# gligen/GLIGEN

Hardware: AMD Instinct MI355X
Metric: 512x512 images/sec @ 50 PLMS steps, box+text (CFG 7.5), UNet step ms (higher is better)
Workload: dtype bf16; 1 GPU; C2: box+text, 8 boxes (30 grounding tokens), 512x512, 50 PLMS steps, CFG 7.5, bf16 storage / fp32 accumulate; plms_steps=50, unet_evals_per_image=102, hipgraph=True, batches_in_flight=3

## Files before the change

gligen_amd/_lib.py:

```python
from __future__ import annotations

import ctypes as C
from pathlib import Path

_HERE = Path(__file__).resolve().parent
LIB_PATH = _HERE / "libgligen_amd.so"


class GligenAmdError(RuntimeError):
    pass


class UNetConfig(C.Structure):
    _fields_ = [
        ("in_channels", C.c_int), ("out_channels", C.c_int), ("model_channels", C.c_int),
        ("num_res_blocks", C.c_int), ("num_heads", C.c_int), ("context_dim", C.c_int),
        ("n_mult", C.c_int), ("channel_mult", C.c_int * 8),
        ("n_attn", C.c_int), ("attention_resolutions", C.c_int * 8),
        ("inpaint_mode", C.c_int), ("grounding_kind", C.c_int),
        ("gr_in_dim", C.c_int), ("gr_out_dim", C.c_int), ("max_persons", C.c_int), ("fuser_kind", C.c_int),
        ("extra_channels", C.c_int), ("tok_resize", C.c_int), ("tok_in_dim", C.c_int),
    ]


# ... 186 lines not shown
TRAIN_PRIM_SYMBOLS = {
    "gl_op_train_attention": (_I, [_P, _I, _I, _I, _I, _I] + [_P] * 9 + [_P]),
    "gl_op_train_linear": (_I, [_P, _I, _I, _I] + [_P] * 8 + [_P]),
    "gl_op_train_layernorm": (_I, [_P, _I, _I, _F, _P, _P, _P, _P, _I] + [_P] * 6 + [_P]),
    "gl_op_train_groupnorm": (_I, [_P, _I, _I, _I, _I, _F, _P, _P, _P, _P, _I] + [_P] * 4 + [_P]),
    "gl_op_train_geglu": (_I, [_P, _I, _I, _P, _P, _P, _P, _P]),
    "gl_op_train_dot": (_I, [_P, C.c_int64, _P, _P, _P, _F, _I, _P, _P]),
    "gl_op_train_conv3": (_I, [_P] + [_I] * 6 + [_P] * 6 + [_P]),
    "gl_op_train_conv_direct": (_I, [_P] + [_I] * 7 + [_P] * 7 + [_P]),
}

class LoraAdapter(C.Structure):
    _fields_ = [("name", C.c_char_p), ("down", C.c_void_p), ("up", C.c_void_p), ("g_down", C.c_void_p), ("g_up", C.c_void_p), ("rank", C.c_int),
                ("scale", C.c_float)]


TRAIN_LORA_SYMBOLS = {
    "gl_unet_train_step_lora": (_I, [_P, C.POINTER(UNetConfig), C.POINTER(TrainUNetIn), _I, C.POINTER(C.c_char_p), C.POINTER(_P), C.POINTER(_P),
                                     C.POINTER(LoraAdapter), _I, _P, _P, _P]),
    "gl_op_lora_linear": (_I, [_P, _I, _I, _I, _I, _F, _I, _I] + [_P] * 10 + [_P]),
    "gl_lora_wgrad_chunk_rows": (_I, [_I]),
}

TRAIN_LORA_CONV_SYMBOLS = {
    "gl_op_lora_conv3": (_I, [_P, _I, _I, _I, _I, _I, _I, _F, _I] + [_P] * 10 + [_P]),
}

TRAINER_SYMBOLS = {
    "gl_op_adamw_ema_step": (_I, [_P, _P, _P, _P, _P, _P, C.c_int64, C.c_double, C.c_double, C.c_double, C.c_double, C.c_double, C.c_double, _I, _P]),
}

_D = C.c_double
TRAIN_RUN_SYMBOLS = {
    "gl_op_grad_accumulate": (_I, [_P, _P, _P, C.c_int64, _I, _I, _P]),
    "gl_grad_sqnorm_partials": (C.c_int64, [C.c_int64]),
    "gl_op_grad_sqnorm": (_I, [_P, _P, C.c_int64, _P, _P]),
    "gl_op_clip_coef": (_I, [_P, _P, C.c_int64, C.c_float, _P, _P]),
    "gl_op_adamw_clip_step": (_I, [_P, _P, _P, _P, _P, C.c_int64, _D, _D, _D, _D, _D, _I, _P, _P]),
    "gl_op_adamw_ema_clip_step": (_I, [_P, _P, _P, _P, _P, _P, C.c_int64, _D, _D, _D, _D, _D, _D, _I, _P, _P]),
    "gl_train_set_loss_weights": (_I, [_P, _P, _I]),
}
GRAD_ACCUM_MODES = {"first": 0, "middle": 1, "last": 2}

SAMPLER_SYMBOLS = {
    "gl_set_cfg_shared_prefix": (_I, [_I]),
}

SOLVER_SYMBOLS = {
    "gl_sample_solver": (_I, [_P, C.POINTER(SolverArgs), _P]),
    "gl_op_solver_update": (_I, [_P, _P, _I, C.c_float, C.c_float, _P, _P, _P, _P, _P, _P] + [C.c_float] * 5 + [C.c_int64, _P]),
}


class GemmPlanRecord(C.Structure):
    _fields_ = [("kernel", C.c_char * 96)] + [(n, C.c_int) for n in ("family", "M", "N", "K", "tm", "tn", "splits", "grid", "n_items", "box", "rm", "rz",
                                                                     "units_per_split", "xcd")]


class AttnProjLayout(C.Structure):
    _fields_ = [(n, C.c_int) for n in ("d", "dp", "dpv", "tq", "tk", "tq_pad", "tk_pad", "vt_perm32")]


class GemmEpilogueArgs(C.Structure):
    _fields_ = [("struct_size", C.c_uint), ("conv", _I), ("M", _I), ("N", _I), ("K", _I), ("x0", _P), ("x1", _P)] + \
               [(n, _I) for n in ("C0", "C1", "B", "H", "W", "stride", "ups", "pad_lo")] + \
               [("w", _P), ("bias", _P), ("bias2", _P), ("bias2_ld", _I), ("rows_per_b", _I), ("res", _P), ("ldres", _I), ("gate", _P)] + \
               [(n, _I) for n in ("act", "out_f32", "mode", "n_real", "remap_in", "remap_out", "remap_off")] + [("out", _P), ("ldo", _I)]


GEMM_PLAN_SYMBOLS = {
    "gl_op_attention_project_range": (_I, [_P, _P, _I, _I, _I, _I, _I, _P, _P, _P, _P, _P, _P, _P, C.POINTER(AttnProjLayout), _P]),
    "gl_op_gemm_epilogue": (_I, [_P, C.POINTER(GemmEpilogueArgs), _P]),
    "gl_gemm_force_plan": (_I, [_I, _I, _I, _I]),
    "gl_gemm_force_knobs": (_I, [_I, _I, _I, _I, _I, _I]),
    "gl_gemm_force_clear": (_I, []),
    "gl_gemm_plan_log_clear": (_I, []),
    "gl_gemm_plan_log": (_I, [C.POINTER(GemmPlanRecord), _I, C.POINTER(_I), C.POINTER(_I)]),
    "gl_op_attention_project": (_I, [_P, _P, _P, _I, _I, _I, _I, _I, _I, _P, _P, _P, _P, _P, _P, C.POINTER(AttnProjLayout), _P]),
}

ATTENTION_CORE_SYMBOLS = {
    "gl_op_attention_core": (_I, [_P, _P, _P, _P, C.POINTER(AttnProjLayout), _I, _I, _I, _I, _P, _I, _I, _I, _P]),
}
ATTN_CORE_KERNELS = {"auto": 0, "attn_kernel": 1, "attn2_kernel_w4": 2, "attn2_kernel_w8": 3, "attn3_kernel": 4}
GL_ERR_UNSUPPORTED = 5


class FFRowsArgs(C.Structure):
    _fields_ = [("struct_size", C.c_uint), ("M", _I), ("C", _I), ("x", _P), ("ldx", _I), ("normalize", _I), ("eps", C.c_float), ("gamma", _P), ("beta", _P),
                ("w1", _P), ("b1", _P), ("w2", _P), ("b2", _P), ("res", _P), ("ldres", _I), ("gate", _P), ("out", _P), ("ldo", _I), ("stats_out", _P),
                ("stats_ld", _I), ("pre", _I), ("post", _I), ("pre_w", _P), ("pre_b", _P), ("pre_res", _P), ("ld_pre_res", _I), ("pre_gate", _P),
                ("mid_out", _P), ("ld_mid", _I), ("post_w", _P), ("post_b", _P), ("post_res", _P), ("ld_post_res", _I), ("gamma_q", _P), ("beta_q", _P),
                ("q", _P), ("qDP", _I), ("qT", _I), ("qTpad", _I)]


class QkvRowsArgs(C.Structure):
    _fields_ = [("struct_size", C.c_uint), ("M", _I), ("C", _I), ("H", _I), ("x", _P), ("ldx", _I), ("normalize", _I), ("eps", C.c_float), ("pre", _I),
                ("pre_w", _P), ("pre_b", _P), ("pre_res", _P), ("ld_pre_res", _I), ("mid_out", _P), ("ld_mid", _I), ("stats_out", _P), ("gamma", _P),
                ("beta", _P), ("np", _I), ("w", _P), ("bias", _P), ("q", _P), ("k", _P), ("vt", _P), ("DP", _I), ("DPV", _I), ("T", _I), ("Tpad_q", _I),
                ("Tpad_k", _I), ("in_period", _I)]


FFN_ROWS_SYMBOLS = {
    "gl_op_ff_rows": (_I, [_P, C.POINTER(FFRowsArgs), _P]),
    "gl_op_qkv_rows": (_I, [_P, C.POINTER(QkvRowsArgs), _P]),
}

class LayerNormRowsArgs(C.Structure):
    _fields_ = [("struct_size", C.c_uint), ("x", _P), ("x2", _P), ("B", _I), ("N1", _I), ("N2", _I), ("Tpad", _I), ("C", _I), ("eps", C.c_float),
                ("gamma", _P), ("beta", _P), ("y", _P), ("ldx", _I), ("ldy", _I)]


NORM_SYMBOLS = {
    "gl_op_groupnorm_coef": (_I, [_P, _P, _I, _P, _I, _I, _I, _P, _P, C.c_float, _P, C.POINTER(_I), _P]),
    "gl_op_layernorm_rows": (_I, [_P, C.POINTER(LayerNormRowsArgs), _P]),
}

VAE_SYMBOLS = {
    "gl_vae_set_attention": (_I, [_P, _I]),
    "gl_op_vae_attention": (_I, [_P, _P, _P, _P, _I, _I, _I, _I, _P, _P]),
}
VAE_ATTN_MODES = {"auto": 0, "matrix": 1, "flash": 2}

LATENT_SYMBOLS = {
    "gl_op_latent_renoise": (_I, [_P, _P, _I, _I, _I, _I, _P, _I, _I, _I, _F, _F, _P, _I, _P]),
    "gl_latent_resize_taps": (_I, [_I, _I, _I, C.POINTER(_I), C.POINTER(_F)]),
}
LATENT_RESIZE_MODES = {"nearest-exact": 0, "bilinear": 1, "bicubic": 2}

LORA_SYMBOLS = {
    "gl_op_lora_merge": (_I, [_P, _P, _P, _P, _I, _I, _I, _F, _P]),
}



class TilePlan(C.Structure):
    _fields_ = [("struct_size", C.c_uint)] + [(n, C.c_int) for n in ("ny", "nx", "th_in", "tw_in", "th_out", "tw_out")] + \
               [(n, C.c_void_p) for n in ("windows", "oy", "ox", "wy", "wx")]


TILING_SYMBOLS = {
    "gl_vae_decode_tiled": (_I, [_P, _I, _I, _I, _P, _P, C.POINTER(TilePlan), _I, _P]),
    "gl_vae_encode_tiled": (_I, [_P, _I, _I, _I, _P, _P, _P, _P, C.POINTER(TilePlan), _I, _P]),
    "gl_op_tile_gather": (_I, [_P, _P, _I, _I, _I, _I, _P, _I, _P, _I, _I, _P]),
    "gl_op_tile_blend": (_I, [_P, _P, _I, _I, C.POINTER(TilePlan), _P, _I, _I, _I, _I, _P]),
}

FUSER_KINDS = {"gatedSA": 0, "gatedSA2": 1, "gatedCA": 2}


def fuser_kind(fuser_type) -> int:
    try:
        return FUSER_KINDS[fuser_type or "gatedSA"]
    except KeyError:
        raise ValueError(f"fuser_type {fuser_type!r}: one of {sorted(FUSER_KINDS)}") from None


_lib = None


def load() -> C.CDLL:
    global _lib
    if _lib is not None:
        return _lib
    if not LIB_PATH.exists():
        raise GligenAmdError(
            f"{LIB_PATH} not found: build it with `python -m gligen_amd.build` "
            "(gligen_amd has no fallback path without its HIP library)")
    import torch
    lib = C.CDLL(str(LIB_PATH))
    for name, (res, args) in {**SYMBOLS, **IMAGE_SYMBOLS, **MAP_SYMBOLS, **TRAIN_MAP_SYMBOLS, **TRAIN_INPUT_SYMBOLS, **TRAIN_FUSER_SYMBOLS, **TRAIN_PRIM_SYMBOLS,
                              **TRAINER_SYMBOLS, **SAMPLER_SYMBOLS, **SOLVER_SYMBOLS, **GEMM_PLAN_SYMBOLS, **ATTENTION_CORE_SYMBOLS, **FFN_ROWS_SYMBOLS, **NORM_SYMBOLS, **VAE_SYMBOLS, **LATENT_SYMBOLS, **LORA_SYMBOLS, **TILING_SYMBOLS, **TRAIN_LORA_SYMBOLS, **TRAIN_LORA_CONV_SYMBOLS,
                              **TRAIN_RUN_SYMBOLS}.items():
        fn = getattr(lib, name)
        fn.restype = res
        fn.argtypes = args
    _lib = lib
    return lib


def check(rc: int) -> None:
    if rc != 0:
        msg = load().gl_last_error()
        raise GligenAmdError(f"libgligen_amd error {rc}: {msg.decode() if msg else '?'}")
```

gligen_amd/build.py:

```python
from __future__ import annotations

import os
import shutil
import subprocess
import sys
from concurrent.futures import ThreadPoolExecutor
from pathlib import Path

HERE = Path(__file__).resolve().parent
CSRC = HERE / "csrc"
INCLUDE = HERE.parent / "include"
LIB = HERE / "libgligen_amd.so"
GEMM_UNITS = ["gemm_u.hip", "gemm_halo.hip", "gemm_wide.hip", "gemm_basic.hip", "gemm.hip"]
SOURCES = [*GEMM_UNITS, "gemm_plan.hip", "ffn.hip", "attention.hip", "vae_attention.hip", "clip.hip", "norm.hip", "misc.hip", "image.hip", "latent.hip", "tile.hip", "lora.hip", "classmap.hip", "convnext.hip",
           "train_ops.hip", "train_attention.hip", "train_layers.hip", "train_spatial.hip", "train_unet.hip", "train_inputs.hip", "train_fusers.hip", "train_optim.hip", "train_lora.hip", "train_lora_conv.hip", "train_run.hip",
           "engine.hip", "engine_unet.hip", "engine_policy.hip", "engine_vae.hip", "engine_clip.hip", "engine_spatial.hip", "engine_sampler.hip", "capi.hip"]
EXTRA_FLAGS = {"attention.hip": ["-mllvm", "-amdgpu-mfma-vgpr-form"], "ffn.hip": ["-fno-slp-vectorize", "-fno-honor-nans"]}
FLAGS = ["--offload-arch=gfx950", "-O3", "-std=c++17", "-fPIC", "-Wall", "-Wno-unused-function"]


def _hipcc() -> str:
    exe = shutil.which("hipcc") or "/opt/rocm/bin/hipcc"
    if not os.path.exists(exe):
        raise RuntimeError("hipcc not found: the gfx950 kernels cannot be built")
    return exe


def _stale() -> bool:
    if not LIB.exists():
        return True
    lib_m = LIB.stat().st_mtime
    deps = list(CSRC.glob("*.hip")) + list(CSRC.glob("*.h")) + list(CSRC.glob("*.inc")) + list(INCLUDE.glob("*.h"))
    return any(p.stat().st_mtime > lib_m for p in deps)


def build_native(force: bool = False, verbose: bool = False) -> Path:
    if not force and not _stale():
        return LIB
    hipcc = _hipcc()
    objdir = HERE / "build"
    objdir.mkdir(exist_ok=True)

    def compile_one(src: str) -> Path:
        obj = objdir / (src + ".o")
        cmd = [hipcc, *FLAGS, *EXTRA_FLAGS.get(src, []), "-I", str(INCLUDE), "-c", str(CSRC / src), "-o", str(obj)]
        r = subprocess.run(cmd, capture_output=True, text=True)
        if r.returncode != 0:
            raise RuntimeError(f"hipcc failed on {src}:\n{r.stderr}")
        if verbose and r.stderr.strip():
            print(r.stderr, file=sys.stderr)
        return obj

    with ThreadPoolExecutor(max_workers=min(len(SOURCES), os.cpu_count() or 4, 16)) as ex:
        objs = list(ex.map(compile_one, SOURCES))
    cmd = [hipcc, "--offload-arch=gfx950", "-shared", "-fPIC", "-o", str(LIB), *map(str, objs)]
    r = subprocess.run(cmd, capture_output=True, text=True)
    if r.returncode != 0:
        raise RuntimeError(f"link failed:\n{r.stderr}")
    build_kbench()
    return LIB


def build_kbench() -> Path:
    exe = HERE / "build" / "kbench"
    cmd = [_hipcc(), *FLAGS, "-I", str(INCLUDE), str(CSRC / "kbench.hip"), "-o", str(exe),
           "-L", str(HERE), "-lgligen_amd", "-Wl,-rpath,$ORIGIN/.."]
    r = subprocess.run(cmd, capture_output=True, text=True)
    if r.returncode != 0:
        raise RuntimeError(f"kbench build failed:\n{r.stderr}")
    return exe


if __name__ == "__main__":
    print(build_native(force="--force" in sys.argv, verbose=True))
```

gligen_amd/csrc/capi.hip:

```cpp
#include "classmap.h"
#include "engine_impl.h"
#include "image.h"
#include "latent.h"
#include "lora.h"
#include "tile.h"
#include "train.h"
#include "train_fusers.h"
#include "../../include/gligen_amd_train_maps.h"
#include "../../include/gligen_amd_train_inputs.h"
#include "../../include/gligen_amd_train_fusers.h"
#include "../../include/gligen_amd_train_prims.h"
#include "../../include/gligen_amd_train_lora.h"
#include "../../include/gligen_amd_train_lora_conv.h"
#include "../../include/gligen_amd_trainer.h"
#include "../../include/gligen_amd_train_run.h"
#include "train_run.h"
#include "../../include/gligen_amd_sampler.h"
#include "../../include/gligen_amd_gemm_plans.h"
#include "../../include/gligen_amd_attention_core.h"
#include "../../include/gligen_amd_ffn_rows.h"
#include "../../include/gligen_amd_norm.h"
#include "../../include/gligen_amd_vae.h"
#include "../../include/gligen_amd_latent.h"
#include "../../include/gligen_amd_lora.h"
#include "../../include/gligen_amd_tiling.h"
#include "gemm_plan.h"

#include <cstdlib>

#include <cmath>

using namespace gl;

struct gl_ctx {
    std::shared_ptr<Engine> holder;
    Engine* eng;
    ImageStage image_stage;
};

#define GL_API_BEGIN try {
#define GL_API_END                                       \
    }                                                    \
    catch (const gl::GlError& e) {                       \
        return gl::set_error(e.code, "%s", e.what());    \
    }                                                    \
    catch (const std::exception& e) {                    \
        return gl::set_error(GL_ERR_STATE, "%s", e.what()); \
    }                                                    \
    return GL_OK;

struct DeviceGuard {
    int prev = -1;
    bool ok = true;
    explicit DeviceGuard(int dev) {
        if (hipGetDevice(&prev) != hipSuccess) prev = -1;
        if (prev != dev) ok = hipSetDevice(dev) == hipSuccess;
        else prev = -1;
    }
    ~DeviceGuard() {
        if (prev >= 0) (void)hipSetDevice(prev);
    }
};
#define NEED(ctx)                                                         \
    if (!(ctx) || !(ctx)->eng) return gl::set_error(GL_ERR_ARG, "null context"); \
    DeviceGuard device_guard_((ctx)->eng->device());                      \
    if (!device_guard_.ok) return gl::set_error(GL_ERR_HIP, "hipSetDevice(%d) failed", (ctx)->eng->device());

static inline hipStream_t S(gl_stream s) { return reinterpret_cast<hipStream_t>(s); }
#define HIPCK_API(expr)                                                                           \
    do {                                                                                          \
        hipError_t _e = (expr);                                                                   \
        if (_e != hipSuccess) throw GlError(GL_ERR_HIP, std::string(#expr) + ": " + hipGetErrorString(_e)); \
    } while (0)

extern "C" {

const char* gl_last_error(void) { return gl::last_error(); }

int gl_ctx_create(int device, size_t arena_bytes, gl_ctx** out) {
    if (!out) return gl::set_error(GL_ERR_ARG, "null out pointer");
    GL_API_BEGIN
    int ndev = 0;
    hipError_t e = hipGetDeviceCount(&ndev);
    if (e != hipSuccess || ndev <= 0)
        throw GlError(GL_ERR_HIP, "no HIP device available: libgligen_amd has no CPU path");
    if (device < 0 || device >= ndev) throw GlError(GL_ERR_ARG, "device index out of range");
    if (hipSetDevice(device) != hipSuccess) throw GlError(GL_ERR_HIP, "hipSetDevice failed");
    hipDeviceProp_t prop;
    if (hipGetDeviceProperties(&prop, device) != hipSuccess) throw GlError(GL_ERR_HIP, "hipGetDeviceProperties failed");
    if (std::string(prop.gcnArchName).rfind("gfx950", 0) != 0)
        throw GlError(GL_ERR_UNSUPPORTED, std::string("libgligen_amd is built for gfx950 (MI355X); device is ") + prop.gcnArchName);
    std::shared_ptr<Engine> eng(new Engine(device));
    eng->arena().init(arena_bytes ? arena_bytes : (size_t(8) << 30));
    eng->init_workspace();
    *out = new gl_ctx{eng, eng.get(), {}};
    GL_API_END
}

int gl_ctx_fork(gl_ctx* parent, size_t arena_bytes, gl_ctx** out) {
    NEED(parent);
    if (!out) return gl::set_error(GL_ERR_ARG, "null out pointer");
    GL_API_BEGIN
// ... 379 lines not shown
int gl_ff_rows_policy_report(char* buf, size_t cap) { return gl::ff_rows_policy_report(buf, cap); }

int gl_set_cfg_shared_prefix(int on) { return gl::cfg_shared_prefix_set(on); }

int gl_vae_set_attention(gl_ctx* ctx, int mode) {
    NEED(ctx);
    GL_API_BEGIN
    ctx->eng->set_vae_attention(mode);
    GL_API_END
}

int gl_op_vae_attention(gl_ctx* ctx, const void* q, const void* k, const void* v, int B, int T, int C, int mode, void* out, gl_stream s) {
    NEED(ctx);
    if (!q || !k || !v || !out) return gl::set_error(GL_ERR_ARG, "gl_op_vae_attention: null pointer");
    GL_API_BEGIN
    if (((reinterpret_cast<uintptr_t>(q) | reinterpret_cast<uintptr_t>(k) | reinterpret_cast<uintptr_t>(v) | reinterpret_cast<uintptr_t>(out)) & 15) != 0)
        throw GlError(GL_ERR_ARG, "gl_op_vae_attention: q, k, v and out are 16-byte aligned");
    ctx->eng->op_vae_attention((const bf16*)q, (const bf16*)k, (const bf16*)v, B, T, C, mode, (bf16*)out, S(s));
    GL_API_END
}

int gl_vae_decode_tiled(gl_ctx* ctx, int B, int h, int w, const float* z, float* img, const gl_tile_plan* plan, int tiles_per_pass, gl_stream s) {
    NEED(ctx);
    if (!z || !img || !plan || B <= 0 || h <= 0 || w <= 0) return gl::set_error(GL_ERR_ARG, "bad vae_decode_tiled arguments");
    GL_API_BEGIN
    ctx->eng->vae_decode_tiled(B, h, w, z, img, *plan, tiles_per_pass, S(s));
    GL_API_END
}

int gl_vae_encode_tiled(gl_ctx* ctx, int B, int H, int W, const float* img, const float* noise, float* z, float* moments_out,
                        const gl_tile_plan* plan, int tiles_per_pass, gl_stream s) {
    NEED(ctx);
    if (!img || !noise || !z || !plan || B <= 0 || H <= 0 || W <= 0) return gl::set_error(GL_ERR_ARG, "bad vae_encode_tiled arguments");
    GL_API_BEGIN
    ctx->eng->vae_encode_tiled(B, H, W, img, noise, z, moments_out, *plan, tiles_per_pass, S(s));
    GL_API_END
}

int gl_op_tile_gather(gl_ctx* ctx, const float* src, int B, int C, int H, int W, const int* windows, int n, float* dst, int TH, int TW, gl_stream s) {
    NEED(ctx);
    return gl::tile_gather_launch(src, B, C, H, W, windows, n, dst, TH, TW, S(s));
}

int gl_op_tile_blend(gl_ctx* ctx, const float* tiles, int first_tile, int n, const gl_tile_plan* plan, float* out, int B, int C, int H, int W,
                     gl_stream s) {
    NEED(ctx);
    if (!plan) return gl::set_error(GL_ERR_ARG, "gl_op_tile_blend: null plan");
    if (plan->struct_size != sizeof(gl_tile_plan))
        return gl::set_error(GL_ERR_ARG, "gl_op_tile_blend: plan->struct_size is %u, this library's gl_tile_plan has %zu bytes", plan->struct_size,
                             sizeof(gl_tile_plan));
    const gl::TileBlendPlan bp{plan->ny, plan->nx, plan->th_out, plan->tw_out, plan->oy, plan->ox, plan->wy, plan->wx};
    return gl::tile_blend_launch(tiles, first_tile, n, bp, out, B, C, H, W, S(s));
}

int gl_gemm_force_plan(int tm, int tn, int splits, int grid_cap) {
    bool tile = tm == 0 && tn == 0;
    for (int c = 0; c < kGemmTiles; ++c) tile |= kGemmTm[c] == tm && kGemmTn[c] == tn;
    if (!tile || splits < 0 || splits > 32 || grid_cap < 0)
        return gl::set_error(GL_ERR_ARG, "gl_gemm_force_plan: tile %dx%d / %d splits / cap %d (tiles 4x5 4x4 2x5 2x4 2x2 or 0x0, splits 0..32, cap >= 0)", tm, tn, splits, grid_cap);
    gemm_force_cfg(tm, tn, tm ? splits : 0);
    gemm_force_grid(grid_cap);
    return GL_OK;
}
int gl_gemm_force_knobs(int halo_splits, int wide_splits, int wide_xcd, int xcd_boxes, int halo, int wide) {
    if (halo_splits < 0 || wide_splits < 0 || wide_xcd < -1 || wide_xcd > 1 || xcd_boxes < 0 || xcd_boxes > 1 || halo < 0 || wide < 0 || wide > 2)
        return gl::set_error(GL_ERR_ARG, "gl_gemm_force_knobs: halo_splits %d, wide_splits %d, wide_xcd %d, xcd_boxes %d, halo %d, wide %d", halo_splits, wide_splits, wide_xcd, xcd_boxes, halo, wide);
    gemm_force_knobs(halo_splits, wide_splits, wide_xcd, xcd_boxes, halo, wide);
    return GL_OK;
}
int gl_gemm_force_clear(void) { gemm_force_clear(); return GL_OK; }
int gl_gemm_plan_log_clear(void) { gemm_plan_log_clear(); return GL_OK; }
int gl_gemm_plan_log(gl_gemm_plan_record* out, int max, int* n_written, int* n_launches) {
    if (!out || !n_written || !n_launches || max < 0) return gl::set_error(GL_ERR_ARG, "gl_gemm_plan_log: null pointer or negative max");
    GemmLogEntry e[kGemmLogSize];
    const int n = gemm_plan_log(e, std::min(max, (int)kGemmLogSize), n_launches);
    for (int i = 0; i < n; ++i) {
        const GemmPlan& p = e[i].plan;
        gl_gemm_plan_record& r = out[i];
        r = gl_gemm_plan_record{};
        snprintf(r.kernel, sizeof r.kernel, "%s", p.name);
        r.family = p.family; r.M = e[i].M; r.N = e[i].N; r.K = e[i].K;
        r.tm = p.tm; r.tn = p.tn; r.splits = p.splits; r.grid = p.grid;
        if (p.family == GEMM_HALO) { r.n_items = p.halo.n_items; r.units_per_split = p.halo.chunks_per_split; }
        else if (p.family == GEMM_WIDE) { r.n_items = p.wide.n_items; r.units_per_split = p.wide.kt_per_split; r.xcd = p.wide.xcd; }
        else {
            r.n_items = p.work.n_items; r.units_per_split = p.work.kt_per_split;
            if (p.family != GEMM_GLDS) { r.box = p.work.box; r.rm = p.work.rm; r.rz = p.work.rz; }
        }
    }
    *n_written = n;
    return GL_OK;
}

int gl_box_calibrate(gl_ctx* ctx, gl_box_calibration* out, gl_stream s) {
    NEED(ctx);
    if (!out) return gl::set_error(GL_ERR_ARG, "gl_box_calibrate: null out pointer");
    GL_API_BEGIN
    Arena& ar = ctx->eng->arena();
    const size_t mk = ar.mark();
    const size_t bytes = size_t(1) << 30;
    void* scratch = ar.alloc(bytes);
    HIPCK_API(hipMemsetAsync(scratch, 1, bytes, S(s)));
    float v[3] = {0.f, 0.f, 0.f};
    int rc = box_calibrate_launch(scratch, bytes, v, S(s));
    ar.release(mk);
    if (rc != GL_OK) throw GlError(rc, gl::last_error());
    out->hbm_copy_gbs = v[0];
    out->lds_dma_tbs = v[1];
    out->mfma_bf16_tflops = v[2];
    GL_API_END
}

int gl_mfma_calibrate(gl_ctx* ctx, int shape, int waves_per_simd, int n_acc, int zero_data, float target_ms, gl_mfma_calibration* out, gl_stream s) {
    NEED(ctx);
    if (!out) return gl::set_error(GL_ERR_ARG, "gl_mfma_calibrate: null out pointer");
    GL_API_BEGIN
    Arena& ar = ctx->eng->arena();
    const size_t mk = ar.mark();
    void* scratch = ar.alloc(4096);
    HIPCK_API(hipMemsetAsync(scratch, 0, 4096, S(s)));
    float v[4] = {0.f, 0.f, 0.f, 0.f};
    int rc = mfma_calibrate_launch(shape, waves_per_simd, n_acc, zero_data, target_ms, scratch, v, S(s));
    ar.release(mk);
    if (rc != GL_OK) throw GlError(rc, gl::last_error());
    out->tflops = v[0];
    out->sclk_mhz = v[1];
    out->ms = v[2];
    out->cycles_per_mfma = v[3];
    GL_API_END
}

int gl_op_linear(gl_ctx* ctx, const void* x, const void* w, const float* bias, const void* res, void* y,
                 int M, int N, int K, int act, int out_f32, gl_stream s) {
    NEED(ctx);
    GL_API_BEGIN
    Epilogue E = e_rows_res(y, N, bias, (const bf16*)res);
    E.out_f32 = out_f32; E.act = act;
    int r = gemm_launch(a_rows((const bf16*)x, K), (const bf16*)w, M, N, K, E, ctx->eng->splitk_ws(), ctx->eng->splitk_ws_bytes(), S(s));
    if (r != GL_OK) throw GlError(r, gl::last_error());
    GL_API_END
}

int gl_op_geglu(gl_ctx* ctx, const void* x, const float* w_f32, const float* b_f32, void* y, int M, int inner, int K, gl_stream s) {
    NEED(ctx);
    GL_API_BEGIN
    Arena& ar = ctx->eng->arena();
    ar.reset();
    bf16* wp = ar.get<bf16>((size_t)2 * inner * K);
    float* bp = ar.get<float>((size_t)2 * inner);
    const int layout = gl::gemm_geglu_layout();
    int r = pack_geglu_launch(w_f32, b_f32, wp, bp, inner, K, layout, S(s));
    if (r != GL_OK) throw GlError(r, gl::last_error());
    Epilogue E = e_rows(y, inner, bp);
    E.act = ACT_GEGLU; E.geglu16 = layout;
    r = gemm_launch(a_rows((const bf16*)x, K), wp, M, 2 * inner, K, E, ctx->eng->splitk_ws(), ctx->eng->splitk_ws_bytes(), S(s));
    if (r != GL_OK) throw GlError(r, gl::last_error());
    GL_API_END
}

int gl_op_ln_linear(gl_ctx* ctx, const void* a, int M, int K0, const float* w0, const float* b0, const void* res, int C,
                    const float* gamma, const float* beta, const float* w1, const float* b1, int mode, int inner_or_heads, int T,
                    void* x_out, void* y_out, int* used_fold, gl_stream s) {
    NEED(ctx);
    if (!a || !w0 || !gamma || !beta || !w1 || !x_out || !y_out || !used_fold) return gl::set_error(GL_ERR_ARG, "gl_op_ln_linear: null pointer");
    GL_API_BEGIN
    Engine& eng = *ctx->eng;
// ... 912 lines not shown
    int r = attn_dims(d, &dp, &dpv);
    if (r != GL_OK) throw GlError(r, gl::last_error());
    const int vt_layout = attn_vt_layout(d, Nk, &dpv);
    *layout = gl_attn_proj_layout{d, dp, dpv, round_up(Nq, 64), round_up(Nk, 64), round_up(round_up(Nq, 64), 128), round_up(Nk, 64), vt_layout};
    if (!q && !k && !vt) return GL_OK;
    if (!xq || !xkv || !wq || !wk || !wv || !q || !k || !vt) throw GlError(GL_ERR_ARG, "gl_op_attention_project: null pointer");
    eng.arena().reset();
    attention_project(eng, xq, xkv, B, Nq, Nk, C, Ck, H, wq, wk, wv, (bf16*)q, (bf16*)k, (bf16*)vt, layout->tq_pad, layout->tk_pad, dp, dpv, vt_layout, S(s));
    GL_API_END
}

int gl_op_attention_project_range(gl_ctx* ctx, const void* x, int B, int Tr, int tok_off, int C, int H, const float* wq, const float* wk,
                                  const float* wv, const float* bias, void* q, void* k, void* vt, const gl_attn_proj_layout* layout, gl_stream s) {
    NEED(ctx);
    if (!x || !wq || !wk || !wv || !q || !k || !vt || !layout) return gl::set_error(GL_ERR_ARG, "gl_op_attention_project_range: null pointer");
    if (B < 1 || Tr < 64 || Tr % 64 || tok_off < 0 || tok_off % 64 || H <= 0 || C % H != 0 || layout->d != C / H)
        return gl::set_error(GL_ERR_ARG, "gl_op_attention_project_range: B=%d Tr=%d tok_off=%d C=%d H=%d d=%d (Tr, tok_off multiples of 64, d = C / H)", B, Tr, tok_off, C, H, layout->d);
    if (tok_off + Tr > layout->tq_pad || tok_off + Tr > layout->tk_pad)
        return gl::set_error(GL_ERR_ARG, "gl_op_attention_project_range: tokens [%d, %d) do not fit tq_pad=%d / tk_pad=%d", tok_off, tok_off + Tr, layout->tq_pad, layout->tk_pad);
    GL_API_BEGIN
    Engine& eng = *ctx->eng;
    int dp, dpv;
    int r = attn_dims(layout->d, &dp, &dpv);
    if (r != GL_OK) throw GlError(r, gl::last_error());
    if (dp != layout->dp || layout->dpv < layout->d) throw GlError(GL_ERR_ARG, "gl_op_attention_project_range: layout->dp / dpv are not this head size's");
    Arena& ar = eng.arena();
    ar.reset();
    auto ck = [&](int rc) { if (rc != GL_OK) throw GlError(rc, gl::last_error()); };
    bf16* wqkv = ar.get<bf16>((size_t)3 * C * C);
    ck(cast_f32_bf16_launch(wq, wqkv, (int64_t)C * C, S(s)));
    ck(cast_f32_bf16_launch(wk, wqkv + (size_t)C * C, (int64_t)C * C, S(s)));
    ck(cast_f32_bf16_launch(wv, wqkv + (size_t)2 * C * C, (int64_t)C * C, S(s)));
    Epilogue E = e_heads(EPI_QKV_HEADS, (bf16*)q, (bf16*)k, C, H, layout->d, dp, Tr, layout->tq_pad, layout->tk_pad);
    E.vt = (bf16*)vt; E.DPV = layout->dpv; E.tok_off = tok_off; E.vt_perm32 = layout->vt_perm32;
    E.bias = bias;
    ck(gemm_launch(a_rows((const bf16*)x, C), wqkv, B * Tr, 3 * C, C, E, eng.splitk_ws(), eng.splitk_ws_bytes(), S(s)));
    GL_API_END
}

int gl_op_gemm_epilogue(gl_ctx* ctx, const gl_gemm_epilogue_args* a, gl_stream s) {
    NEED(ctx);
    if (!a) return gl::set_error(GL_ERR_ARG, "gl_op_gemm_epilogue: null args");
    if (a->struct_size != sizeof(gl_gemm_epilogue_args))
        return gl::set_error(GL_ERR_ARG, "gl_op_gemm_epilogue: args->struct_size is %u, this library's gl_gemm_epilogue_args has %zu bytes", a->struct_size,
                             sizeof(gl_gemm_epilogue_args));
    if (!a->x0 || !a->w || !a->out || (a->C1 && !a->x1)) return gl::set_error(GL_ERR_ARG, "gl_op_gemm_epilogue: null pointer (x0, w, out; x1 when C1 > 0)");
    GL_API_BEGIN
    Engine& eng = *ctx->eng;
    Arena& ar = eng.arena();
    ar.reset();
    AOperand A{};
    const bf16* w = (const bf16*)a->w;
    int M = a->M, K = a->K;
    if (a->conv) {
        const int Cin = a->C0 + a->C1;
        if (a->N < 1 || Cin < 1 || a->B < 1 || a->H < 1 || a->W < 1 || a->ups < 0 || a->ups > 1 || (a->stride != 1 && a->stride != 2))
            throw GlError(GL_ERR_ARG, "gl_op_gemm_epilogue: conv geometry");
        bf16* wp = ar.get<bf16>((size_t)a->N * 9 * Cin);
        int r = pack_conv_weight_launch((const float*)a->w, wp, a->N, Cin, 3, 3, a->N, S(s));
        if (r != GL_OK) throw GlError(r, gl::last_error());
        w = wp;
        const int Hup = a->H << a->ups, Wup = a->W << a->ups;
        const int Ho = a->stride == 1 ? Hup : (a->pad_lo ? (Hup + 2 - 3) / 2 + 1 : (Hup + 1 - 3) / 2 + 1);
        const int Wo = a->stride == 1 ? Wup : (a->pad_lo ? (Wup + 2 - 3) / 2 + 1 : (Wup + 1 - 3) / 2 + 1);
        A.p0 = (const bf16*)a->x0; A.C0 = a->C0; A.ld0 = a->C0; A.p1 = (const bf16*)a->x1; A.C1 = a->C1; A.ld1 = a->C1;
        A.mode = A_CONV3; A.Hin = a->H; A.Win = a->W; A.Ho = Ho; A.Wo = Wo; A.stride = a->stride; A.ups = a->ups; A.pad_lo = a->pad_lo;
        M = a->B * Ho * Wo; K = 9 * Cin;
    } else {
        A = a_rows((const bf16*)a->x0, K);
    }
    if (a->mode != EPI_ROWMAJOR && a->mode != EPI_NCHW_F32) throw GlError(GL_ERR_ARG, "gl_op_gemm_epilogue: mode is 0 (row-major) or 3 (NCHW fp32)");
    Epilogue E;
    epilogue_defaults(E);
    E.mode = a->mode; E.act = a->act; E.out = a->out; E.ldo = a->ldo; E.out_f32 = a->out_f32;
    E.bias = a->bias; E.bias2 = a->bias2; E.bias2_ld = a->bias2_ld; E.rows_per_b = a->rows_per_b;
    E.res = (const bf16*)a->res; E.ldres = a->ldres; E.gate = a->gate;
    E.n_real = a->n_real;
    E.remap_in = a->remap_in; E.remap_out = a->remap_out; E.remap_off = a->remap_off;
    int r = gemm_launch(A, w, M, a->N, K, E, eng.splitk_ws(), eng.splitk_ws_bytes(), S(s));
    if (r != GL_OK) throw GlError(r, gl::last_error());
    GL_API_END
}

int gl_op_attention_core(gl_ctx* ctx, const void* q, const void* k, const void* vt, const gl_attn_proj_layout* layout, int B, int H, int Nq,
                         int Nk, void* o, int ldo, int o_rows_per_b, int kernel, gl_stream s) {
    NEED(ctx);
    if (!q || !k || !vt || !o || !layout) return gl::set_error(GL_ERR_ARG, "gl_op_attention_core: null pointer");
    GL_API_BEGIN
    const gl_attn_proj_layout& L = *layout;
    int dp, dpv;
    int r = attn_dims(L.d, &dp, &dpv);
    if (r != GL_OK) throw GlError(r, gl::last_error());
    if (B <= 0 || H <= 0 || L.dp != dp) throw GlError(GL_ERR_ARG, "gl_op_attention_core: B, H > 0 and dp = 48 / 80 / 160 for d = 40 / 80 / 160");
    if (ldo < H * L.d || ldo % 4 != 0 || o_rows_per_b < Nq || (reinterpret_cast<uintptr_t>(o) & 7) != 0)
        throw GlError(GL_ERR_ARG, "gl_op_attention_core: ldo >= H d, ldo % 4 == 0, o_rows_per_b >= Nq, o 8-byte aligned");
    if (((reinterpret_cast<uintptr_t>(q) | reinterpret_cast<uintptr_t>(k) | reinterpret_cast<uintptr_t>(vt)) & 15) != 0)
        throw GlError(GL_ERR_ARG, "gl_op_attention_core: q, k and vt are 16-byte aligned");
    if (L.vt_perm32 != 0 && L.vt_perm32 != 1) throw GlError(GL_ERR_ARG, "gl_op_attention_core: vt_perm32 is 0 or 1");
    if (kernel == ATTN_SEL_AUTO && L.dpv != (L.vt_perm32 && L.d == 40 ? 48 : dpv))
        throw GlError(GL_ERR_ARG, "gl_op_attention_core: dpv does not belong to (d, vt_perm32)");
    AttnParams P = attn_params((const bf16*)q, (const bf16*)k, (const bf16*)vt, (bf16*)o, H, L.d, Nq, Nk, L.tq_pad, L.tk_pad, L.vt_perm32);
    P.ldo = ldo;
    P.o_rows_per_b = o_rows_per_b;
    P.counters = ctx->eng->attn_counters();
    r = attn_launch_select(P, B, L.dpv, kernel, S(s));
    if (r != GL_OK) throw GlError(r, gl::last_error());
    GL_API_END
}

int gl_attn_regime_counters(gl_ctx* ctx, int enable, unsigned* lazy_moves, unsigned* reruns) {
    NEED(ctx);
    if (!lazy_moves || !reruns) return gl::set_error(GL_ERR_ARG, "gl_attn_regime_counters: null pointer");
    GL_API_BEGIN
    unsigned c[ATTN_CTR_N];
    ctx->eng->attn_regime_counters(enable, c);
    *lazy_moves = c[ATTN_CTR_LAZY_MOVES];
    *reruns = c[ATTN_CTR_RERUNS];
    GL_API_END
}


int gl_op_proj_attention(gl_ctx* ctx, const void* x, int B, int N, int C, int H, const float* pre_w, const float* pre_b, const void* pre_res,
                         const float* gamma, const float* beta, const float* wq, const float* wk, const float* wv, int Nkv_extra,
                         void* mid, void* o, int* used_rows, gl_stream s) {
    NEED(ctx);
    if (!x || !pre_w || !pre_b || !gamma || !beta || !wq || !wk || !wv || !mid || !o || !used_rows)
        return gl::set_error(GL_ERR_ARG, "gl_op_proj_attention: null pointer");
    GL_API_BEGIN
    Engine& eng = *ctx->eng;
    Arena& ar = eng.arena();
    ar.reset();
    auto ck = [&](int rc) { if (rc != GL_OK) throw GlError(rc, gl::last_error()); };
    if (C % H != 0 || N % 64 != 0 || Nkv_extra != 0) throw GlError(GL_ERR_ARG, "gl_op_proj_attention: C % H == 0, N % 64 == 0");
    const int d = C / H, M = B * N;
    int dp, dpv;
    ck(attn_dims(d, &dp, &dpv));
    const int vt_layout = attn_vt_layout(d, N, &dpv);
    AttnBufs& bufs = eng.attn_bufs(B, H, d, N, N, dpv);
    bf16* wqkv = ar.get<bf16>((size_t)3 * C * C);
    float* bias = ar.get<float>((size_t)3 * C);
    {
        float* wf = ar.get<float>((size_t)C * C);
        const float* ws[3] = {wq, wk, wv};
        for (int i = 0; i < 3; ++i) {
            ck(ln_fold_launch(ws[i], nullptr, gamma, beta, wf, bias + (size_t)i * C, C, C, S(s)));
            ck(cast_f32_bf16_launch(wf, wqkv + (size_t)i * C * C, (int64_t)C * C, S(s)));
        }
    }
    const bool want = *used_rows != 0;
    const bool rows = want && qkv_rows_supported(M, C, d, N) && vt_layout == 1;
    *used_rows = rows ? 1 : 0;
    if (rows) {
        void* st = ar.alloc(qkv_rows_stream_bytes(C, true, 3));
        ck(qkv_rows_pack_launch(pre_w, wqkv, 3, st, C, S(s)));
        QkvRowsParams P{};
        P.x = (const bf16*)x; P.ldx = C; P.eps = 1e-5f; P.stream = st; P.M = M;
        P.pre = 1; P.pre_b = pre_b; P.pre_res = (const bf16*)pre_res; P.ld_pre_res = C; P.mid_out = (bf16*)mid; P.ld_mid = C;
        P.np = 3; P.bias = bias; P.q = bufs.q; P.k = bufs.k; P.vt = bufs.vt;
        P.H = H; P.d = d; P.DP = dp; P.DPV = dpv; P.T = N; P.Tpad_q = bufs.Tq_pad; P.Tpad_k = bufs.Tk_pad; P.vt_perm32 = vt_layout;
        ck(qkv_rows_launch(P, C, S(s)));
    } else {
        bf16* pw = ar.get<bf16>((size_t)C * C);
        ck(cast_f32_bf16_launch(pre_w, pw, (int64_t)C * C, S(s)));
        {
            ck(gemm_launch(a_rows((const bf16*)x, C), pw, M, C, C, e_rows_res(mid, C, pre_b, (const bf16*)pre_res), eng.splitk_ws(), eng.splitk_ws_bytes(), S(s)));
        }
// ... 133 lines not shown
```

gligen_amd/csrc/engine.hip:

```cpp
#include "engine_impl.h"

#include <algorithm>
#include <cmath>
#include <cstdarg>
#include <cstring>

namespace gl {

static thread_local char g_err[2048] = "";
int set_error(int code, const char* fmt, ...) {
    va_list ap;
    va_start(ap, fmt);
    vsnprintf(g_err, sizeof(g_err), fmt, ap);
    va_end(ap);
    return code;
}
const char* last_error() { return g_err; }

void Arena::init(size_t bytes) {
    off_ = hw_ = 0;
    HIPCK(hipGetDevice(&dev_));
    int vmm = 0;
    const char* sw = dev_env("GL_ARENA_VMM");
    if (!(sw && atoi(sw) == 0) && hipDeviceGetAttribute(&vmm, hipDeviceAttributeVirtualMemoryManagementSupported, dev_) == hipSuccess && vmm) {
// ... 382 lines not shown
                f.chain_q_stream = cq;
                f.chain_q_bias = qb;
            }
        }
    }
    return f;
}

ResW Engine::resw(const std::string& p, int Cin, int Cout, bool unet) {
    ResW r;
    r.Cin = Cin;
    r.Cout = Cout;
    if (unet) {
        r.n1 = norm(p + ".in_layers.0");
        r.c1 = conv3(p + ".in_layers.2");
        r.n2 = norm(p + ".out_layers.0");
        r.c2 = conv3(p + ".out_layers.3");
        r.has_skip = has(p + ".skip_connection.weight");
        if (r.has_skip) r.skip = conv1(p + ".skip_connection");
    } else {
        r.n1 = norm(p + ".norm1");
        r.c1 = conv3(p + ".conv1");
        r.n2 = norm(p + ".norm2");
        r.c2 = conv3(p + ".conv2");
        r.has_skip = has(p + ".nin_shortcut.weight");
        if (r.has_skip) r.skip = conv1(p + ".nin_shortcut");
        if (has(p + ".conv_shortcut.weight")) throw GlError(GL_ERR_UNSUPPORTED, "'" + p + "': 3x3 conv_shortcut is not supported");
    }
    if (r.c1.Cin != Cin || r.c1.Cout != Cout || (Cin != Cout) != r.has_skip)
        throw GlError(GL_ERR_ARG, fmt("'%s': weights do not match the configured topology (%d -> %d)", p.c_str(), Cin, Cout));
    return r;
}

void Engine::finalize() {
    if (finalized_) throw GlError(GL_ERR_STATE, "gl_finalize called twice");
    HIPCK(hipSetDevice(device_));
    if (unet_.present) build_unet();
    if (vae_.dec.present) build_vae();
    if (vae_.dec.present && has("vae/encoder.conv_in.weight")) build_vae_encoder();
    if (clipt_.present) build_clip_text();
    if (clipv_.present) build_clip_vision();
    HIPCK(hipDeviceSynchronize());
    for (void* p : fold_tmps_) (void)hipFree(p);
    fold_tmps_.clear();
    for (auto it = raw_.begin(); it != raw_.end();) {
        if (it->second.shape.size() >= 2 && it->first.find("quant_conv") == std::string::npos && !keep_raw_.count(it->first)) {
            (void)hipFree(it->second.p);
            it = raw_.erase(it);
        } else {
            ++it;
        }
    }
    finalized_ = true;
}

FILE* launch_log_file() {
    static FILE* f = dev_env("GL_LAUNCH_LOG") ? fopen(dev_env("GL_LAUNCH_LOG"), "w") : nullptr;
    return f;
}
AttnParams attn_params(const bf16* q, const bf16* k, const bf16* vt, bf16* o, int H, int d, int Nq, int Nk, int Tq_pad, int Tk_pad, int vt_layout) {
    AttnParams P{};
    P.q = q; P.k = k; P.vt = vt; P.o = o;
    P.H = H; P.d = d; P.Nq = Nq; P.Nk = Nk; P.Tq_pad = Tq_pad; P.Tk_pad = Tk_pad;
    P.ldo = H * d; P.o_rows_per_b = Nq; P.vt_layout = vt_layout;
    P.scale_log2e = (float)(1.4426950408889634 / std::sqrt((double)d));
    return P;
}

void Engine::attention(const bf16* q, const bf16* k, const bf16* vt, bf16* o, int B, int H, int d, int Nq, int Nk, int Tq_pad, int Tk_pad, int vt_layout,
                       hipStream_t s) {
    const AttnParams P = attn_params(q, k, vt, o, H, d, Nq, Nk, Tq_pad, Tk_pad, vt_layout);
    const char* sym = attn_kernel_name(d, Nk, vt_layout);
    {
        ProfScope ps(this, s, sym, 4.0 * B * H * (double)Nq * Nk * d, 0.0);
        CK(attn_launch(P, B, s));
        if (FILE* f = launch_log_file()) {
            fprintf(f, "%s|%d|%d|%d|2|%.0f\n", sym, Nq, Nk, d, 2.0 * B * H * d * (2.0 * Nq + 2.0 * Nk));
            fflush(f);
        }
    }
    ++n_launches;
}

void Engine::gemm(const AOperand& A, const bf16* W, int M, int N, int K, const Epilogue& E, hipStream_t s) {
    ProfScope ps(this, s, "gemm", 2.0 * M * N * K, 0.0);
    CK(gemm_launch(A, W, M, N, K, E, ws_, ws_bytes_, s));
    if (profiling_) {
        static const bool by_shape = dev_env("GL_PROF_SHAPES") != nullptr;
        std::string nm = gemm_last_kernel_name();
        if (by_shape) nm += fmt(" M%d N%d K%d", M, N, K);
        ps.rename(nm);
    }
    FILE* launch_log = launch_log_file();
    if (launch_log) {
        const double a_rows = A.mode != A_ROWS ? (double)(M / (A.Ho * A.Wo)) * A.Hin * A.Win : (double)M;
        const double out_b = E.mode == EPI_NCHW_F32 ? 4.0 * M * E.n_real : (E.act == ACT_GEGLU ? 1.0 : 2.0) * M * (double)N * (E.out_f32 ? 2 : 1);
        const double bytes = a_rows * (A.C0 + A.C1) * 2 + (double)N * K * 2 + out_b + (E.res ? 2.0 * M * N : 0.0);
        fprintf(launch_log, "%s|%d|%d|%d|%d|%.0f\n", gemm_last_kernel_name(), M, N, K, A.mode, bytes);
        fflush(launch_log);
    }
    {
        int tm, tn, sp;
        gemm_last_cfg(&tm, &tn, &sp);
        n_launches += sp > 1 ? 2 : 1;
    }
}

bf16* Engine::linear_rows(const bf16* x, int M, const LinW& L, int act, const bf16* res, const float* gate, hipStream_t s, RowStats* stats) {
    bf16* out = arena_.get<bf16>((size_t)M * L.N);
    Epilogue E = e_rows_res(out, L.N, L.b, res);
    E.act = act;
    E.gate = gate;
    if (stats) {
        *stats = RowStats{};
        if (ln_fold_ && L.N % 64 == 0) {
            stats->ld = L.N / 32;
            stats->p = arena_.get<float2>((size_t)M * stats->ld);
            E.stats_out = stats->p;
            E.stats_ld = stats->ld;
        }
    }
    gemm(a_rows(x, L.K), L.w, M, L.N, L.K, E, s);
    if (stats && stats->p) stats->nb = gemm_last_stats_nb();
    return out;
}

bf16* Engine::groupnorm(const TRef& x, int B, int HW, const NormW& n, float eps, bool silu, hipStream_t s) {
    const int C = x.C();
    if (n.C != C) throw GlError(GL_ERR_ARG, fmt("groupnorm: %d channels given to a norm with %d", C, n.C));
    bf16* y = arena_.get<bf16>((size_t)B * HW * C);
    GNParams P{};
    P.x0 = x.p0; P.C0 = x.C0; P.x1 = x.p1; P.C1 = x.C1;
    P.B = B; P.HW = HW; P.eps = eps; P.gamma = n.g; P.beta = n.b; P.y = y; P.silu = silu ? 1 : 0;
    P.partial = reinterpret_cast<float*>(arena_.alloc(gn_partial_bytes(B, HW)));
    ProfScope ps(this, s, HW <= 256 ? "gn_small_kernel" : "gn_stats_kernel + gn_apply_kernel", 0.0, 2.0 * B * HW * (double)C * 2);
    CK(groupnorm_launch(P, s));
    n_launches += HW <= 256 ? 1 : 2;
    return y;
}

bf16* Engine::gn_silu_conv3x3(const TRef& x, int B, int H, int W, const NormW& n, float eps, const ConvW& c, const float* bias2, int bias2_ld,
                              const bf16* res, bf16* out, hipStream_t s) {
    if (x.C() != c.Cin || n.C != c.Cin) throw GlError(GL_ERR_ARG, fmt("gn_silu_conv3x3: %d channels into a norm of %d and a conv of %d", x.C(), n.C, c.Cin));
    const int HW = H * W, M = B * HW;
    if (!out) out = arena_.get<bf16>((size_t)M * c.Cout);
    AOperand A = a_conv3(x, H, W, H, W, 1, 0, 1);
    Epilogue E = e_rows_res(out, c.Cout, c.b, res);
    E.bias2 = bias2; E.bias2_ld = bias2_ld; E.rows_per_b = HW;
    if (gn_prologue_ && gemm_gn_prologue_supported(A, M, c.Cout, 9 * c.Cin, E)) {
        GNParams P{};
        P.x0 = x.p0; P.C0 = x.C0; P.x1 = x.p1; P.C1 = x.C1;
        P.B = B; P.HW = HW; P.eps = eps; P.gamma = n.g; P.beta = n.b; P.silu = 1;
        P.partial = reinterpret_cast<float*>(arena_.alloc(gn_partial_bytes(B, HW)));
        P.coef = reinterpret_cast<float*>(arena_.alloc(gn_coef_bytes(B, c.Cin)));
        {
            const int nl = groupnorm_coef_launches(HW, x.C0, x.C1);
            ProfScope ps(this, s, nl == 1 ? "gn_small_coef_kernel" : "gn_stats_kernel + gn_coef_kernel", 0.0, 1.0 * B * HW * (double)c.Cin * 2);
            CK(groupnorm_coef_launch(P, s));
            n_launches += nl;
        }
        A.gn = P.coef;
        gemm(A, c.w, M, c.Cout, 9 * c.Cin, E, s);
        ++n_prologue_convs;
        return out;
    }
    bf16* a = groupnorm(x, B, HW, n, eps, true, s);
    A.p0 = a; A.C0 = c.Cin; A.ld0 = c.Cin; A.p1 = nullptr; A.C1 = 0; A.ld1 = 0;
    gemm(A, c.w, M, c.Cout, 9 * c.Cin, E, s);
// ... 122 lines not shown
```

gligen_amd/csrc/gemm.h:

```cpp
#pragma once
#include "common.h"

namespace gl {

enum { A_ROWS = 0, A_CONV3 = 1, A_CONV2UP = 2 };

struct AOperand {
    const bf16* p0;
    const bf16* p1;
    int C0, C1;
    int ld0, ld1;
    int mode;
    int Hin, Win, Ho, Wo;
    int stride, ups, pad_lo;
    const float* gn = nullptr;
};

enum { EPI_ROWMAJOR = 0, EPI_QK_HEADS = 1, EPI_VT_HEADS = 2, EPI_NCHW_F32 = 3, EPI_QKV_HEADS = 4 };
enum { ACT_NONE = 0, ACT_SILU = 1, ACT_GEGLU = 2, ACT_GELU = 3, ACT_QUICK_GELU = 4 };

struct Epilogue {
    int mode;
    int act;
    void* out;
    int ldo;
    int out_f32;
    const float* bias;
    const float* bias2;
    int bias2_ld;
    int rows_per_b;
    unsigned rpb_magic;
    int rpb_shift;
    const bf16* res;
    int ldres;
    const float* gate;
    bf16* q;
    bf16* k;
    int q_tiled;
    int C, H, d, DP, T;
    int Tpad_q, Tpad_k;
    bf16* vt;
    int DPV;
    int tok_off;
    int vt_perm32;
    int n_real;
    int remap_in, remap_out, remap_off;
    int up_win;
    int geglu16;
    float2* stats_out;
    int stats_ld;
    const float2* ln_stats;
    int ln_nb, ln_ld;
    const float* ln_csum;
    float ln_inv_c, ln_eps;
};

__host__ __device__ inline size_t ktile_off(size_t bh, int tpad, int t, int dd, int DP) {
    return (bh * (size_t)tpad + (size_t)(t & ~63)) * DP + (size_t)(dd >> 3) * 512 + (size_t)(t & 63) * 8 + (dd & 7);
}

int gemm_launch(const AOperand& A, const bf16* W, int M, int N, int K, const Epilogue& E,
                float* ws, size_t ws_bytes, hipStream_t stream);

int gemm_launch_t(const bf16* Wrows, int Mw, const bf16* X, int Nx, int K, const Epilogue& E,
                  hipStream_t stream);

void epilogue_defaults(Epilogue& E);
bool gemm_supports_qkv();
void gemm_set_variant(int v);
int gemm_geglu_layout();
void gemm_force_cfg(int tm, int tn, int splits);
void gemm_force_grid(int blocks);
void gemm_set_autotune(int on);
void gemm_set_no_split(int on);
void gemm_set_plan_batch_scale(int scale);
void gemm_last_cfg(int* tm, int* tn, int* splits);
const char* gemm_last_kernel_name();
bool gemm_gn_prologue_supported(const AOperand& A, int M, int N, int K, const Epilogue& E);
bool gemm_upconv_phases_supported(const AOperand& A, int M, int N, int K, const Epilogue& E);
bool gemm_ln_fold_supported(const AOperand& A, int M, int N, int K, const Epilogue& E);
int gemm_last_stats_nb();
void aoperand_rows(AOperand& A, const bf16* p, int K, int ld);

}
```

gligen_amd/csrc/gemm.hip:

```cpp
#include "gemm_impl.h"

#include <algorithm>
#include <climits>
#include <cstdio>
#include <cstdlib>
#include <cstring>

namespace gl {

void epilogue_defaults(Epilogue& E) {
    E = Epilogue{};
    E.mode = EPI_ROWMAJOR;
    E.act = ACT_NONE;
    E.rows_per_b = 1;
    E.rpb_magic = 1; E.rpb_shift = 0;
}

void aoperand_rows(AOperand& A, const bf16* p, int K, int ld) {
    A = AOperand{};
    A.p0 = p;
    A.C0 = K;
    A.ld0 = ld;
    A.mode = A_ROWS;
}
// ... 27 lines not shown
                val[0] += a.x; val[1] += a.y; val[2] += a.z; val[3] += a.w;
                gate[0] += b.x; gate[1] += b.y; gate[2] += b.z; gate[3] += b.w;
            }
            epi_geglu4(E, m, n0, val, gate);
        } else {
            const bool fast = E.mode == EPI_ROWMAJOR && !E.out_f32 && !E.remap_in && E.act != ACT_GELU && E.act != ACT_QUICK_GELU && !E.ln_stats;
            const float4 pb = *reinterpret_cast<const float4*>((fast && E.bias) ? E.bias + n0 : ws);
            const float4 pb2 = *reinterpret_cast<const float4*>((fast && E.bias2) ? E.bias2 + (size_t)div_rpb(E, m) * E.bias2_ld + n0 : ws);
            const uint2 pr = *reinterpret_cast<const uint2*>((fast && E.res) ? reinterpret_cast<const void*>(E.res + (size_t)m * E.ldres + n0)
                                                                              : reinterpret_cast<const void*>(ws));
            const float pg = *((fast && E.res && E.gate) ? E.gate : ws);
            float v[4] = {0, 0, 0, 0};
            const float* p0 = ws + (size_t)m * N + n0;
            const size_t zs = (size_t)M * N;
            for (int z = 0; z < splits; z += 4) {
                float4 a[4];
#pragma unroll
                for (int u = 0; u < 4; ++u) a[u] = *reinterpret_cast<const float4*>(p0 + (size_t)min(z + u, splits - 1) * zs);
#pragma unroll
                for (int u = 0; u < 4; ++u) {
                    const bool ok = z + u < splits;
                    v[0] += ok ? a[u].x : 0.f; v[1] += ok ? a[u].y : 0.f; v[2] += ok ? a[u].z : 0.f; v[3] += ok ? a[u].w : 0.f;
                }
            }
            if (E.ln_stats) {
                const float2 st = ln_row_stats(E, m);
                const float4 cs = *reinterpret_cast<const float4*>(E.ln_csum + n0);
                v[0] = st.y * (v[0] - st.x * cs.x); v[1] = st.y * (v[1] - st.x * cs.y);
                v[2] = st.y * (v[2] - st.x * cs.z); v[3] = st.y * (v[3] - st.x * cs.w);
            }
            if (fast) {
                if (E.bias) { v[0] += pb.x; v[1] += pb.y; v[2] += pb.z; v[3] += pb.w; }
                if (E.bias2) { v[0] += pb2.x; v[1] += pb2.y; v[2] += pb2.z; v[3] += pb2.w; }
                if (E.act == ACT_SILU) {
#pragma unroll
                    for (int i = 0; i < 4; ++i) v[i] = silu_f(v[i]);
                }
                if (E.res) {
                    U2BF4 r;
                    r.u = pr;
                    const float g = E.gate ? pg : 1.f;
#pragma unroll
                    for (int i = 0; i < 4; ++i) v[i] = bf2f(r.e[i]) + g * v[i];
                }
                int mo = m;
                if (E.up_win) {
                    const int mp = M >> 2, ph = m / mp, r = m - ph * mp, q = div_rpb(E, r);
                    mo = ((2 * q + (ph >> 1)) * E.up_win + (r - q * E.up_win)) * 2 + (ph & 1);
                }
                store_bf16x4(reinterpret_cast<bf16*>(E.out) + (size_t)mo * E.ldo + n0, v);
            } else {
                epi_finish4(E, m, n0, v);
            }
        }
    }
}

static thread_local GemmPlan t_last = [] { GemmPlan p{}; strcpy(p.name, "gemm"); return p; }();
int gemm_last_stats_nb() { return t_last.stats_nb; }
const char* gemm_last_kernel_name() { return t_last.name; }
void gemm_last_cfg(int* tm, int* tn, int* splits) { *tm = t_last.tm; *tn = t_last.tn; *splits = t_last.splits; }
static thread_local GemmLogEntry t_log[kGemmLogSize];
static thread_local int t_log_n = 0;
void gemm_plan_log_clear() { t_log_n = 0; }
int gemm_plan_log(GemmLogEntry* out, int max, int* launches) {
    if (launches) *launches = t_log_n;
    const int n = std::max(0, std::min(std::min(t_log_n, kGemmLogSize), max));
    for (int i = 0; i < n; ++i) out[i] = t_log[(t_log_n - n + i) % kGemmLogSize];
    return n;
}

namespace {

int execute(const GemmPlan& p, const AOperand& A, const bf16* W, int M, int N, int K, const Epilogue& E_in, float* ws, hipStream_t stream) {
    Epilogue E = E_in;
    if ((p.family == GEMM_P || p.family == GEMM_U) && !p.stats_nb) E.stats_out = nullptr;
    const Launch l{A, W, M, N, K, E, ws, stream};
    switch (p.family) {
        case GEMM_GLDS:
        case GEMM_P: GL_TRY(gemm_exec_basic(l, p)); break;
        case GEMM_U: GL_TRY(gemm_exec_u(l, p)); break;
        case GEMM_HALO: GL_TRY(gemm_exec_halo(l, p)); break;
        case GEMM_WIDE: GL_TRY(gemm_exec_wide(l, p)); break;
        default: return gemm_unknown_tile();
    }
    if (p.splits > 1) {
        int64_t total = (int64_t)M * (N / 4);
        int blocks = (int)fmin((double)cdiv64(total, 256), 4096.0);
        hipLaunchKernelGGL(splitk_reduce_kernel, dim3(blocks), dim3(256), 0, stream, ws, p.splits, M, N, E);
        GL_LAUNCH_CHECK();
    }
    return GL_OK;
}

int tune(const bf16* W, float* ws, hipStream_t stream, const GemmProblem& pb, bool use_u, const char* key, const GemmCand& model, GemmCand* win, bool* cache) {
    hipStreamCaptureStatus cap = hipStreamCaptureStatusNone;
    if (stream) (void)hipStreamIsCapturing(stream, &cap);
    if (cap != hipStreamCaptureStatusNone) return GL_OK;
    auto run = [&](const GemmCand& c, hipStream_t s) -> int {
        GemmPlan plan{};
        GL_TRY(gemm_plan_tile(pb, use_u, c, plan));
        return execute(plan, pb.A, W, pb.M, pb.N, pb.K, pb.E, ws, s);
    };
    GL_HIP(hipDeviceSynchronize());
    hipEvent_t ev[2];
    GL_HIP(hipEventCreate(&ev[0]));
    GL_HIP(hipEventCreate(&ev[1]));
    struct EvGuard { hipEvent_t* e; ~EvGuard() { (void)hipEventDestroy(e[0]); (void)hipEventDestroy(e[1]); } } ev_guard{ev};
    float win_ms = 1e30f;
    const int tune_reps = gemm_knobs().tune_reps, corun = gemm_knobs().corun;
    hipStream_t s2 = nullptr;
    hipEvent_t ev_fork = nullptr, ev_join = nullptr;
    struct CoGuard { hipStream_t& s; hipEvent_t &a, &b; ~CoGuard() { if (a) (void)hipEventDestroy(a); if (b) (void)hipEventDestroy(b); if (s) (void)hipStreamDestroy(s); } } co_guard{s2, ev_fork, ev_join};
    if (corun) {
        GL_HIP(hipStreamCreateWithFlags(&s2, hipStreamNonBlocking));
        GL_HIP(hipEventCreateWithFlags(&ev_fork, hipEventDisableTiming));
        GL_HIP(hipEventCreateWithFlags(&ev_join, hipEventDisableTiming));
    }
    for (const GemmCand& c : gemm_tune_candidates(pb, use_u)) {
        GL_TRY(run(c, stream));
        GL_HIP(hipEventRecord(ev[0], stream));
        if (corun) {
            GL_HIP(hipEventRecord(ev_fork, stream));
            GL_HIP(hipStreamWaitEvent(s2, ev_fork, 0));
            for (int r = 0; r < tune_reps; ++r) {
                GL_TRY(run(c, stream));
                GL_TRY(run(c, s2));
            }
            GL_HIP(hipEventRecord(ev_join, s2));
            GL_HIP(hipStreamWaitEvent(stream, ev_join, 0));
        } else
            for (int r = 0; r < tune_reps; ++r) GL_TRY(run(c, stream));
        GL_HIP(hipEventRecord(ev[1], stream));
        GL_HIP(hipEventSynchronize(ev[1]));
        float ms = 0.f;
        GL_HIP(hipEventElapsedTime(&ms, ev[0], ev[1]));
        if (ms < win_ms) { win_ms = ms; *win = c; }
    }
    *cache = true;
    if (gemm_knobs().tune_log)
        fprintf(stderr, "[gemm autotune] %s -> %dx%d / %d splits @%d (%.1f us; model said %dx%d / %d) cfg %d %d %d\n", key, kGemmTm[win->c] * 32,
                kGemmTn[win->c] * 32, win->sp, win->grid ? win->grid : 512, win_ms * 1e3f / tune_reps, kGemmTm[model.c] * 32, kGemmTn[model.c] * 32, model.sp,
                win->c, win->sp, win->grid);
    return GL_OK;
}

}

int gemm_launch(const AOperand& A, const bf16* W, int M, int N, int K, const Epilogue& E_in, float* ws,
                size_t ws_bytes, hipStream_t stream) {
    t_last.stats_nb = 0;
    Epilogue E = E_in;
    GemmPlan plan;
    GL_TRY(gemm_plan(A, M, N, K, E, ws != nullptr, ws_bytes, plan, [&](auto&&... a) { return tune(W, ws, stream, a...); }));
    t_last = plan;
    t_log[t_log_n % kGemmLogSize] = GemmLogEntry{plan, M, N, K};
    t_log_n = t_log_n == INT_MAX ? kGemmLogSize : t_log_n + 1;
    return execute(plan, A, W, M, N, K, E, ws, stream);
}

int gemm_launch_t(const bf16* Wrows, int Mw, const bf16* X, int Nx, int K, const Epilogue& E, hipStream_t stream) {
    AOperand A;
    aoperand_rows(A, Wrows, K, K);
    return gemm_launch(A, X, Mw, Nx, K, E, nullptr, 0, stream);
}

}
```

gligen_amd/csrc/gemm_impl.h:

```cpp
#pragma once
#include <type_traits>

#include "gemm_plan.h"

namespace gl {

__device__ __forceinline__ int perm_tok4(int t0, int p32 = 0) {
    if (p32) {
        const int g = (t0 >> 2) & 7;
        return (t0 & ~31) | ((((g & 1) << 2) | (g >> 1)) << 2);
    }
    int g = (t0 >> 2) & 3;
    int gp = ((g & 1) << 1) | (g >> 1);
    return (t0 & ~15) | (gp << 2);
}

__device__ __forceinline__ void store_bf16x4(bf16* dst, const float v[4]) {
    U2BF4 o;
    o.e[0] = f2bf(v[0]);
    o.e[1] = f2bf(v[1]);
    o.e[2] = f2bf(v[2]);
    o.e[3] = f2bf(v[3]);
    *reinterpret_cast<uint2*>(dst) = o.u;
}
// ... 179 lines not shown
                        }
                        epi_geglu4(E, m, nv0, val, gate);
                    }
                }
            } else {
#pragma unroll
                for (int q = 0; q < 4; ++q) {
                    int n0 = nb + 8 * q;
                    if (n0 < N) {
                        float v[4];
#pragma unroll
                        for (int e = 0; e < 4; ++e) v[e] = acc[i][j][4 * q + e];
                        epi_finish4(E, m, n0, v);
                    }
                }
            }
        }
    }
}

#define GL_GLDS16(gsrc, ldst)                                                                      \
    __builtin_amdgcn_global_load_lds((const __attribute__((address_space(1))) void*)(gsrc),       \
                                     (__attribute__((address_space(3))) void*)(ldst), 16, 0, 0)

__device__ __forceinline__ void epi_geglu4_t16(const Epilogue& E, int m, int nv0, float val[4], float gate[4]) {
    if (E.bias) {
        float4 bv = *reinterpret_cast<const float4*>(E.bias + nv0);
        float4 bg = *reinterpret_cast<const float4*>(E.bias + nv0 + 16);
        val[0] += bv.x; val[1] += bv.y; val[2] += bv.z; val[3] += bv.w;
        gate[0] += bg.x; gate[1] += bg.y; gate[2] += bg.z; gate[3] += bg.w;
    }
    const int j0 = (nv0 >> 5) * 16 + (nv0 & 15);
    float o[4];
#pragma unroll
    for (int i = 0; i < 4; ++i) o[i] = val[i] * gelu_erf_f(gate[i]);
    store_bf16x4(reinterpret_cast<bf16*>(E.out) + (size_t)m * E.ldo + j0, o);
}

template <int OFF>
__device__ __forceinline__ void lds_rd16(bf16x8& d, unsigned addr) {
    asm volatile("ds_read_b128 %0, %1 offset:%2" : "=v"(d) : "v"(addr), "n"(OFF));
}
template <int N, int STRIDE, int I = 0>
__device__ __forceinline__ void lds_rd16_n(bf16x8 (&d)[N], unsigned addr) {
    if constexpr (I < N) {
        lds_rd16<I * STRIDE>(d[I], addr);
        lds_rd16_n<N, STRIDE, I + 1>(d, addr);
    }
}
__device__ __forceinline__ void epi_ready(float4& v) { asm volatile("" : "+v"(v.x), "+v"(v.y), "+v"(v.z), "+v"(v.w)); }
template <int N>
__device__ __forceinline__ void pin_regs(bf16x8 (&d)[N]) {
#pragma unroll
    for (int i = 0; i < N; ++i) asm volatile("" : "+v"(d[i]));
}

#define GL_BLDS16(rsrc, ldst, voff, soff)                                                                   \
    __builtin_amdgcn_raw_ptr_buffer_load_lds(rsrc, (__attribute__((address_space(3))) void*)(ldst), 16, \
                                             (int)(voff), (int)(soff), 0, 0)

__device__ __forceinline__ float2 ln_row_stats(const Epilogue& E, int m) {
    float s = 0.f, q = 0.f;
    for (int nb = 0; nb < E.ln_nb; ++nb) {
        const float2 v = E.ln_stats[(size_t)m * E.ln_ld + nb];
        s += v.x; q += v.y;
    }
    const float mean = s * E.ln_inv_c;
    const float var = fmaxf(q * E.ln_inv_c - mean * mean, 0.f);
    return make_float2(mean, rsqrtf(var + E.ln_eps));
}

struct Launch {
    const AOperand& A; const bf16* W; int M, N, K; const Epilogue& E; float* ws;
    hipStream_t stream;
    template <auto KFN, class... Tail> int run(dim3 grid, int block, size_t lds, const Tail&... tail) const {
        return launch_lds<KFN>(grid, dim3(block), lds, stream, A, W, M, N, K, E, ws, tail...);
    }
};

int gemm_exec_basic(const Launch& l, const GemmPlan& p);
int gemm_exec_u(const Launch& l, const GemmPlan& p);
int gemm_exec_halo(const Launch& l, const GemmPlan& p);
int gemm_exec_wide(const Launch& l, const GemmPlan& p);
inline int gemm_unknown_tile() { return set_error(GL_ERR_UNSUPPORTED, "gemm: unknown tile candidate"); }

}
```

gligen_amd/csrc/gemm_plan.h:

```cpp
#pragma once
#include <functional>
#include <vector>

#include "gemm.h"

namespace gl {

struct WorkDesc {
    int tiles_n;
    int splits;
    int kt_per_split;
    int n_items;
    int box, rm, rz;
};
struct HaloDesc {
    int tiles_n, splits, chunks_per_split, n_items;
    int lgW, lgH;
};
struct WideDesc {
    int tiles_n, splits, kt_per_split, n_items;
    int xcd;
};

struct GemmKnobs {
    int variant = 4;
    int wide = 1, wide_splits = 0;
    int halo = 8, halo_splits = 0;
    int xcd_boxes = 1, wide_xcd = -1;
    int autotune = 1, tune_reps = 3, corun = 0;
    bool no_table = false, tune_log = false;
    int force_tm = 0, force_tn = 0, force_splits = 0, force_grid = 0;
};
GemmKnobs& gemm_knobs();
void gemm_force_knobs(int halo_splits, int wide_splits, int wide_xcd, int xcd_boxes, int halo, int wide);
void gemm_force_clear();

struct GemmProblem {
    const AOperand& A;
    int M, N, K;
    const Epilogue& E;
    bool has_ws; size_t ws_bytes;
};

enum GemmFamily { GEMM_GLDS, GEMM_P, GEMM_U, GEMM_HALO, GEMM_WIDE };

struct GemmCand { int c, sp, grid; };
constexpr int kGemmTiles = 5;
extern const int kGemmTm[kGemmTiles], kGemmTn[kGemmTiles];

struct GemmPlan {
    int family;
    int tm, tn, amode;
    bool qkv, gn;
    int splits;
    int grid;
    union { WorkDesc work; HaloDesc halo; WideDesc wide; };
    int stats_nb;
    char name[96];
};

struct GemmLogEntry { GemmPlan plan; int M, N, K; };
constexpr int kGemmLogSize = 32;
void gemm_plan_log_clear();
int gemm_plan_log(GemmLogEntry* out, int max, int* launches);

std::vector<GemmCand> gemm_tune_candidates(const GemmProblem& pb, bool use_u);
int gemm_plan_tile(const GemmProblem& pb, bool use_u, const GemmCand& cand, GemmPlan& plan);

using GemmTuner = std::function<int(const GemmProblem& pb, bool use_u, const char* key, const GemmCand& model, GemmCand* win, bool* cache)>;

int gemm_plan(const AOperand& A, int M, int N, int K, Epilogue& E, bool has_ws, size_t ws_bytes, GemmPlan& plan, const GemmTuner& tuner = nullptr);

}
```

gligen_amd/csrc/gemm_plan.hip:

```cpp
#include "gemm_plan.h"

#include <algorithm>
#include <cmath>
#include <cstdio>
#include <mutex>
#include <string>
#include <unordered_map>

namespace gl {

static GemmKnobs read_knobs() {
    static const struct { const char* env; int GemmKnobs::*knob; } kInt[] = {
        {"GL_GEMM_VARIANT", &GemmKnobs::variant}, {"GL_GEMM_WIDE", &GemmKnobs::wide}, {"GL_GEMM_WIDE_SPLITS", &GemmKnobs::wide_splits},
        {"GL_CONV_HALO", &GemmKnobs::halo}, {"GL_CONV_HALO_SPLITS", &GemmKnobs::halo_splits}, {"GL_GEMM_XCD_BOXES", &GemmKnobs::xcd_boxes},
        {"GL_WIDE_XCD", &GemmKnobs::wide_xcd}, {"GL_GEMM_AUTOTUNE", &GemmKnobs::autotune}, {"GL_GEMM_TUNE_REPS", &GemmKnobs::tune_reps},
        {"GL_GEMM_TUNE_CORUN", &GemmKnobs::corun}};
    GemmKnobs k;
    for (const auto& e : kInt)
        if (const char* v = dev_env(e.env)) k.*e.knob = atoi(v);
    k.tune_reps = std::max(1, k.tune_reps);
    k.no_table = dev_env("GL_GEMM_NO_TABLE") != nullptr;
    k.tune_log = dev_env("GL_GEMM_TUNE_LOG") != nullptr;
    return k;
}
GemmKnobs& gemm_knobs() {
    static GemmKnobs k = read_knobs();
    return k;
}
void gemm_set_variant(int v) { gemm_knobs().variant = v < 0 ? read_knobs().variant : v; }
void gemm_set_autotune(int on) { gemm_knobs().autotune = on < 0 ? read_knobs().autotune : on; }
void gemm_force_cfg(int tm, int tn, int splits) { gemm_knobs().force_tm = tm; gemm_knobs().force_tn = tn; gemm_knobs().force_splits = splits; }
void gemm_force_grid(int g) { gemm_knobs().force_grid = g; }
void gemm_force_knobs(int halo_splits, int wide_splits, int wide_xcd, int xcd_boxes, int halo, int wide) {
    GemmKnobs& k = gemm_knobs();
    k.halo_splits = halo_splits; k.wide_splits = wide_splits; k.wide_xcd = wide_xcd; k.xcd_boxes = xcd_boxes; k.halo = halo; k.wide = wide;
}
void gemm_force_clear() {
    const GemmKnobs d = read_knobs();
    gemm_force_cfg(0, 0, 0);
    gemm_force_grid(0);
    gemm_force_knobs(d.halo_splits, d.wide_splits, d.wide_xcd, d.xcd_boxes, d.halo, d.wide);
}
static thread_local int t_no_split = 0;
void gemm_set_no_split(int on) { t_no_split = on; }
static thread_local int t_plan_scale = 1;
void gemm_set_plan_batch_scale(int scale) { t_plan_scale = scale > 1 ? scale : 1; }

int gemm_geglu_layout() { return gemm_knobs().variant >= 2 ? 1 : 0; }
bool gemm_supports_qkv() { return gemm_knobs().variant == 4; }

static size_t a_rows(const AOperand& A, int M) {
    return A.mode != A_ROWS && A.Ho * A.Wo > 0 ? (size_t)(M / (A.Ho * A.Wo)) * A.Hin * A.Win : (size_t)M;
}
static int row_tiles(const AOperand& A, int M, int bm) { return A.mode == A_CONV2UP ? 4 * cdiv(M / 4, bm) : cdiv(M, bm); }
static bool fits_buffer_offsets(const AOperand& A, int M, int N, int K) {
    return a_rows(A, M) * (size_t)std::max(A.ld0, A.ld1) * 2 < 0x7fff0000ull && (size_t)N * K * 2 * (A.mode == A_CONV2UP ? 4 : 1) < 0x7fff0000ull;
}

static inline int ilog2_exact(int v) {
    int l = 0;
    while ((1 << l) < v) ++l;
    return (1 << l) == v ? l : -1;
}
static bool halo_eligible(const AOperand& A, int M, int N, int K, const Epilogue& E) {
    if (A.mode != A_CONV3 || A.stride != 1 || A.ups || A.pad_lo != 1 || A.Ho != A.Hin || A.Wo != A.Win) return false;
    const int lgW = ilog2_exact(A.Win), lgH = ilog2_exact(A.Hin);
    if (lgW < 3 || lgW > 6 || lgH < 0 || M % 256) return false;
    const int R = 256 >> lgW, HB = std::min(A.Hin, R);
    if ((R / HB) * (HB + 2) * (A.Win + 2) > 448) return false;
    if (A.C0 % 64 || A.C1 % 64 || (N % 160 && N % 128)) return false;
    if (E.mode != EPI_ROWMAJOR || E.remap_in || (E.act != ACT_NONE && E.act != ACT_SILU) || (E.bias2 && E.res)) return false;
    if (E.bias2 && (E.rows_per_b != A.Hin * A.Win)) return false;
    return fits_buffer_offsets(A, M, N, K);
}
static bool wide_eligible(const AOperand& A, int M, int N, int K, const Epilogue& E) {
    if (A.mode != A_ROWS || M % 256 || (N % 160 && N % 128)) return false;
    if (A.C1 && A.C0 % 64) return false;
    if (E.mode != EPI_ROWMAJOR || E.remap_in || E.bias2) return false;
    if (E.act == ACT_GEGLU) { if (N % 128 || !E.geglu16 || E.res || E.out_f32) return false; }
    else if (E.act != ACT_NONE && E.act != ACT_SILU) return false;
    return fits_buffer_offsets(A, M, N, K);
}

static int gemm_route(const AOperand& A, int M, int N, int K, const Epilogue& E, bool honour_force = true) {
    const GemmKnobs& kn = gemm_knobs();
    if (A.mode == A_CONV2UP) return kn.variant == 4 && fits_buffer_offsets(A, M, N, K) ? GEMM_U : GEMM_P;
    if (kn.variant < 2 || (N < 128 && E.act != ACT_GEGLU)) return GEMM_GLDS;
    const bool use_u = kn.variant == 4 && fits_buffer_offsets(A, M, N, K) && !(E.bias2 && (E.res || A.mode == A_ROWS));
    if (!use_u) return GEMM_P;
    const bool forced = honour_force && kn.force_tm;
    if (kn.halo && !forced && N >= 128 && halo_eligible(A, M, N, K, E) && M >= kn.halo * 256) return GEMM_HALO;
    if (kn.wide && !forced && (kn.wide >= 2 || E.act == ACT_GEGLU) && wide_eligible(A, M, N, K, E)) return GEMM_WIDE;
    return GEMM_U;
}

bool gemm_gn_prologue_supported(const AOperand& A, int M, int N, int K, const Epilogue& E) {
    return K % 64 == 0 && gemm_route(A, M, N, K, E) == GEMM_HALO && (A.Hin * A.Win) % 256 == 0;
}

bool gemm_upconv_phases_supported(const AOperand& A, int M, int N, int K, const Epilogue& E) {
    if (A.mode != A_CONV2UP || M <= 0 || M != 4 * (M / (4 * A.Hin * A.Win)) * A.Hin * A.Win || A.Ho != 2 * A.Hin || A.Wo != 2 * A.Win) return false;
    if ((A.C0 + A.C1) % 64 || A.C0 % 64 || K != 4 * (A.C0 + A.C1) || N % 8 || A.gn) return false;
    if (E.mode != EPI_ROWMAJOR || E.act != ACT_NONE || E.out_f32 || E.bias2 || E.res || E.gate || E.remap_in || E.stats_out || E.ln_stats) return false;
    return gemm_route(A, M, N, K, E) == GEMM_U;
}

bool gemm_ln_fold_supported(const AOperand& A, int M, int N, int K, const Epilogue& E) {
    if (A.mode != A_ROWS || A.C1 || K % 64) return false;
    if (E.act == ACT_GEGLU) return E.mode == EPI_ROWMAJOR && gemm_route(A, M, N, K, E, false) == GEMM_WIDE;
    if (E.mode != EPI_QKV_HEADS && E.mode != EPI_QK_HEADS) return false;
    Epilogue Eh = E;
    Eh.bias2 = nullptr;
    return gemm_route(A, M, N, K, Eh, false) == GEMM_U;
}

static int gemm_validate(const AOperand& A, int M, int N, int K, Epilogue& E) {
    if (E.rows_per_b < 1) return set_error(GL_ERR_ARG, "gemm: rows_per_b=%d", E.rows_per_b);
    {
        E.up_win = A.mode == A_CONV2UP ? A.Win : 0;
        const unsigned d = E.up_win ? (unsigned)E.up_win : (unsigned)E.rows_per_b;
        int sh = 0;
        while ((1ull << sh) < d) ++sh;
        E.rpb_shift = sh;
        E.rpb_magic = (unsigned)((((1ull << sh) - d) << 32) / d + 1);
    }
    if (M <= 0 || N <= 0 || K <= 0) return set_error(GL_ERR_ARG, "gemm: empty problem M=%d N=%d K=%d", M, N, K);
    if (E.ln_stats && (!E.ln_csum || !E.bias || E.ln_nb < 1 || E.ln_ld < E.ln_nb || !gemm_ln_fold_supported(A, M, N, K, E)))
        return set_error(GL_ERR_UNSUPPORTED, "gemm: folded LayerNorm needs csum + folded bias + statistics, and an epilogue that applies them");
    if (K % 64 != 0) return set_error(GL_ERR_ARG, "gemm: K=%d must be a multiple of 64", K);
    if (N % 4 != 0) return set_error(GL_ERR_ARG, "gemm: N=%d must be a multiple of 4", N);
    if (A.gn && !gemm_gn_prologue_supported(A, M, N, K, E))
        return set_error(GL_ERR_UNSUPPORTED, "gemm: the GroupNorm prologue (AOperand::gn) exists in conv_halo_kernel only (3x3, stride 1, H W %% 256 == 0)");
    if (A.mode == A_CONV2UP) {
        if (!gemm_upconv_phases_supported(A, M, N, K, E))
            return set_error(GL_ERR_UNSUPPORTED, "conv3x3: no phase form of the upsample conv for this launch (gemm_u_kernel, bias-only bf16 epilogue, K = 4 Cin, N %% 8 == 0)");
    } else if (A.mode == A_CONV3) {
        if ((A.C0 + A.C1) % 64 != 0 || A.C0 % 64 != 0 || K != 9 * (A.C0 + A.C1))
            return set_error(GL_ERR_ARG, "conv3x3: channels (%d,%d) must be multiples of 64 and K=9*Cin (K=%d)", A.C0, A.C1, K);
    } else {
        if (K != A.C0 + A.C1 || (A.C1 && A.C0 % 64 != 0))
            return set_error(GL_ERR_ARG, "gemm: K=%d does not match operand channels (%d,%d)", K, A.C0, A.C1);
    }
    if (A.mode != A_ROWS && (E.gate || E.remap_in))
        return set_error(GL_ERR_UNSUPPORTED, "conv3x3: the gated residual and the row remap are row-GEMM epilogues");
    if ((E.act == ACT_GELU || E.act == ACT_QUICK_GELU) && (E.res || E.bias2 || A.mode != A_ROWS))
        return set_error(GL_ERR_UNSUPPORTED, "gemm: the GELU / quick-GELU epilogues have no residual / broadcast-bias form");
    if (E.act == ACT_GEGLU && (N % 32 != 0 || E.mode != EPI_ROWMAJOR))
        return set_error(GL_ERR_ARG, "gemm: GEGLU epilogue needs packed N %% 32 == 0 (N=%d)", N);
    if (E.act == ACT_GEGLU && E.geglu16 != gemm_geglu_layout())
        return set_error(GL_ERR_STATE, "gemm: GEGLU weights were packed for a different main-loop variant");
    if (E.mode == EPI_QKV_HEADS) {
        if (A.mode != A_ROWS || A.C1) return set_error(GL_ERR_ARG, "gemm: EPI_QKV_HEADS takes a single row-major activation operand");
        if (!gemm_supports_qkv() || !fits_buffer_offsets(A, M, N, K) || N != 3 * E.C || (2 * E.C) % 128 || !E.vt || !E.q || !E.k || E.T % 64 || M % E.T)
            return set_error(GL_ERR_UNSUPPORTED, "gemm: EPI_QKV_HEADS needs the v5 main loop, N = 3C with 2C %% 128 == 0, tokens per sample %% 64 == 0");
    }
    return GL_OK;
}

namespace {

struct Cfg { int bm, bn; float speed; };
const Cfg kCfgs[4] = {{128, 128, 1.0f}, {128, 64, 0.8f}, {64, 64, 0.55f}, {128, 32, 0.45f}};

const char* reduce_suffix(int splits) { return splits > 1 ? " + splitk_reduce_kernel" : ""; }
int split_units(const GemmProblem& pb, int want, int tiles, int units, int min_units, bool allowed, int& splits) {
    int sp = want;
    if (sp <= 0) {
        sp = 1;
        while (tiles * sp < 200 && units / (sp * 2) >= min_units) sp *= 2;
    }
    sp = std::max(1, std::min(sp, units));
    if (!pb.has_ws || !allowed) sp = 1;
    while (sp > 1 && (size_t)sp * pb.M * pb.N * sizeof(float) > pb.ws_bytes) --sp;
    const int per = cdiv(units, sp);
    splits = cdiv(units, per);
    return per;
}

void plan_glds(const GemmProblem& pb, const GemmProblem& ph, GemmPlan& p) {
    const int M = ph.M, N = pb.N;
    int best = 0;
    float best_score = -1.f;
    for (int c = 0; c < 4; ++c) {
        if (c == 3 && N > 32) continue;
        if (c != 3 && N <= 32) continue;
        const Cfg& cf = kCfgs[c];
        double tm = cdiv(M, cf.bm), tn = cdiv(N, cf.bn);
        double pad = ((double)M * N) / (tm * cf.bm * tn * cf.bn);
        double fill = fmin(1.0, tm * tn / 256.0);
        float score = (float)(pad * cf.speed * (0.35 + 0.65 * fill));
        if (score > best_score) { best_score = score; best = c; }
    }
    const Cfg& cf = kCfgs[best];
    snprintf(p.name, sizeof p.name, "gemm_glds_kernel<%dx%d, %d>", cf.bm, cf.bn, pb.A.mode);
    const int tiles_h = cdiv(M, cf.bm) * cdiv(N, cf.bn), tiles = cdiv(pb.M, cf.bm) * cdiv(N, cf.bn);
    const int nk = pb.K / 64;
    int splits = 1;
    if (pb.has_ws && !t_no_split && tiles_h < 256 && nk >= 8) {
        splits = std::min(std::min(cdiv(512, tiles_h), nk / 4), 16);
        while (splits > 1 && (size_t)splits * M * N * sizeof(float) > pb.ws_bytes) --splits;
    }
    const int kps = cdiv(nk, splits);
    p.splits = cdiv(nk, kps);
    p.tm = cf.bm / 32; p.tn = cf.bn / 32; p.grid = tiles;
    p.work = WorkDesc{cdiv(N, cf.bn), p.splits, kps, tiles, -1, 0, p.splits};
}

void plan_halo(const GemmProblem& pb, const GemmProblem& ph, GemmPlan& p) {
    const AOperand& A = pb.A;
    const int M = pb.M, N = pb.N, tn = N % 160 == 0 ? 5 : 4;
    HaloDesc& hd = p.halo;
    hd.lgW = ilog2_exact(A.Win); hd.lgH = ilog2_exact(A.Hin);
    hd.tiles_n = cdiv(N, tn * 32);
    const int tiles = (M / 256) * hd.tiles_n;
    hd.chunks_per_split = split_units(ph, gemm_knobs().halo_splits, (ph.M / 256) * hd.tiles_n, (A.C0 + A.C1) / 64, 2, true, hd.splits);
    hd.n_items = tiles * hd.splits;
    p.tm = 8; p.tn = tn; p.gn = A.gn != nullptr; p.splits = hd.splits;
    p.grid = std::min(hd.n_items, 256);
    snprintf(p.name, sizeof p.name, "conv_halo_kernel<%d, %d%s>%s", tn, 8, p.gn ? ", gn" : "", reduce_suffix(p.splits));
}

void plan_wide(const GemmProblem& pb, const GemmProblem& ph, GemmPlan& p) {
    const Epilogue& E = pb.E;
    const int M = pb.M, N = pb.N, tn = (E.act != ACT_GEGLU && N % 160 == 0) ? 5 : 4;
    WideDesc& wd = p.wide;
    wd.tiles_n = N / (tn * 32);
    const int tiles = (M / 256) * wd.tiles_n;
    wd.kt_per_split = split_units(ph, gemm_knobs().wide_splits, (ph.M / 256) * wd.tiles_n, pb.K / 64, 4, E.act != ACT_GEGLU, wd.splits);
    wd.n_items = tiles * wd.splits;
    wd.xcd = gemm_knobs().wide_xcd >= 0 ? gemm_knobs().wide_xcd : (wd.tiles_n % 8 != 0 && wd.n_items >= 512);
    if (wd.n_items < 256 || std::min(wd.n_items, 256) % 8) wd.xcd = 0;
    p.tm = 8; p.tn = tn; p.splits = wd.splits;
    p.grid = std::min(wd.n_items, 256);
    snprintf(p.name, sizeof p.name, "gemm_wide_kernel<%d>%s", tn, reduce_suffix(p.splits));
}

}

const int kGemmTm[kGemmTiles] = {4, 4, 2, 2, 2}, kGemmTn[kGemmTiles] = {5, 4, 5, 4, 2};
static const int kSp[10] = {1, 2, 3, 4, 6, 8, 12, 16, 24, 32};

static bool feasible(const GemmProblem& pb, bool use_u, int c, int& sp) {
    const Epilogue& E = pb.E;
    const int tm = kGemmTm[c], tn = kGemmTn[c], nk = pb.K / 64;
    if (c == 4 && !use_u) return false;
    if (E.act == ACT_GEGLU && (tn & 1)) return false;
    if (E.mode == EPI_QKV_HEADS && (sp > 1 || (2 * E.C) % (tn * 32) || (tm == 4 && tn == 5))) return false;
    if (E.mode == EPI_QK_HEADS && E.ln_stats && (sp > 1 || (tm == 4 && tn == 5))) return false;
    if (sp > 1 && (t_no_split || !pb.has_ws || nk / sp < 2 || (size_t)sp * pb.M * pb.N * sizeof(float) > pb.ws_bytes)) return false;
    sp = cdiv(nk, cdiv(nk, sp));
    return true;
}

static void tuned_key(const GemmProblem& pb, bool use_u, char* key, size_t n) {
    const AOperand& A = pb.A; const Epilogue& E = pb.E;
    snprintf(key, n, "%d,%d,%d|%d,%d,%d,%d,%d,%d,%d|%d,%d,%d,%d,%d,%d|%d%s", pb.M, pb.N, pb.K, A.mode, A.C0, A.C1, A.stride, A.ups, A.Win,
             A.Hin, E.mode, E.act, E.res != nullptr, E.bias2 != nullptr, E.out_f32, E.gate != nullptr, (int)use_u,
             (E.mode == EPI_QK_HEADS && E.ln_stats) ? "|ln" : t_no_split ? "|ns" : "");
}

static bool forced_choice(const GemmProblem& pb, bool use_u, GemmCand& out) {
    const GemmKnobs& kn = gemm_knobs();
    const int want = kn.force_splits ? kn.force_splits : 1;
    if (!kn.force_tm || want < 1 || want > kSp[9]) return false;
    for (int c = 0; c < kGemmTiles; ++c) {
        int sp = want;
        if (kGemmTm[c] != kn.force_tm || kGemmTn[c] != kn.force_tn || !feasible(pb, use_u, c, sp) || sp != want) continue;
        out = GemmCand{c, sp, 0};
        return true;
    }
    return false;
}

static bool model_choice(const GemmProblem& pb, bool use_u, GemmCand& out) {
    const int M = pb.M, N = pb.N, nk = pb.K / 64;
    double best_t = 1e30;
    out = GemmCand{-1, 1, 0};
    for (int c = 0; c < 4; ++c) {
        const int bm = kGemmTm[c] * 32, bn = kGemmTn[c] * 32;
        const int tiles = row_tiles(pb.A, M, bm) * cdiv(N, bn);
        for (int si = 0; si < 10; ++si) {
            int sp = kSp[si];
            if (!feasible(pb, use_u, c, sp)) continue;
            const int kps = cdiv(nk, sp);
            const int items = tiles * sp;
            const int per_block = cdiv(items, 512);
            double t_kt = 0.15 * bm * bn + 500.0;
            if (items <= 256) t_kt *= 0.75;
            const double t_item = kps * t_kt + (pb.E.act == ACT_GEGLU ? 9000.0 : 6000.0) * (bm * bn / 20480.0);
            double tt = per_block * t_item;
            if (sp > 1) tt += 6000.0 + (double)sp * M * N * 8.0 / 2000.0;
            if (tt < best_t) { best_t = tt; out.c = c; out.sp = sp; }
        }
    }
    return out.c >= 0;
}

std::vector<GemmCand> gemm_tune_candidates(const GemmProblem& pb, bool use_u) {
    const int M = pb.M, N = pb.N;
    const bool corun = gemm_knobs().corun;
    std::vector<GemmCand> out;
    for (int c = 0; c < kGemmTiles; ++c) {
        const int tiles = row_tiles(pb.A, M, kGemmTm[c] * 32) * cdiv(N, kGemmTn[c] * 32);
        if (c == 4 && ((size_t)M * N > ((size_t)1 << 23) || N % 64)) continue;
        int last_sp = -1;
        for (int si = 0; si < 10; ++si) {
            int sp = kSp[si];
            if (!feasible(pb, use_u, c, sp) || sp == last_sp) continue;
            last_sp = sp;
            if (sp > 1 && tiles * sp > 4096) continue;
            for (int gi = 0; gi < (corun ? 5 : 3); ++gi) {
                const int grid = gi == 0 ? 0 : gi == 1 ? 768 : gi == 2 ? 1024 : gi == 3 ? 256 : 128;
                if (gi == 1 && (kGemmTm[c] * 32 + kGemmTn[c] * 32 > 192 || tiles * sp <= 512)) continue;
                if (gi == 2 && (kGemmTm[c] * 32 + kGemmTn[c] * 32 > 128 || tiles * sp <= 768)) continue;
                if (gi == 3 && tiles * sp <= 256) continue;
                if (gi == 4 && tiles * sp <= 128) continue;
                out.push_back(GemmCand{c, sp, grid});
// ... 1 lines not shown
        }
    }
    return out;
}

int gemm_plan_tile(const GemmProblem& pb, bool use_u, const GemmCand& cand, GemmPlan& p) {
    const auto& [A, M, N, K, E, has_ws, ws_bytes] = pb;
    const int nk = K / 64;
    if (cand.c < 0 || cand.c >= (use_u ? kGemmTiles : 4)) return set_error(GL_ERR_UNSUPPORTED, "gemm: unknown tile candidate");
    const int tm = kGemmTm[cand.c], tn = kGemmTn[cand.c];
    WorkDesc& wd = p.work;
    wd.tiles_n = cdiv(N, tn * 32);
    wd.kt_per_split = cdiv(nk, cand.sp);
    wd.splits = cdiv(nk, wd.kt_per_split);
    wd.n_items = row_tiles(A, M, tm * 32) * wd.tiles_n * wd.splits;
    wd.box = -1; wd.rm = 0; wd.rz = wd.splits;
    if (use_u && gemm_knobs().xcd_boxes) {
        const int tiles_m = row_tiles(A, M, tm * 32), tiles_n = wd.tiles_n;
        const double a_bytes = (double)a_rows(A, M) * (A.C0 + A.C1) * 2, w_bytes = (double)N * K * 2;
        double best = 1e300;
        for (int lgm = 3; lgm >= 0; --lgm)
            for (int lgn = 3 - lgm; lgn >= 0; --lgn) {
                const int lgz = 3 - lgm - lgn;
                if (tiles_m % (1 << lgm) || tiles_n % (1 << lgn) || wd.splits % (1 << lgz)) continue;
                const double cost = a_bytes * (1 << lgn) + w_bytes * (1 << lgm);
                if (cost < best) {
                    best = cost;
                    wd.box = lgm | lgn << 4;
                    wd.rm = tiles_m >> lgm; wd.tiles_n = tiles_n >> lgn; wd.rz = wd.splits >> lgz;
                }
            }
    }
    p.family = use_u ? GEMM_U : GEMM_P;
    p.tm = tm; p.tn = tn; p.amode = A.mode; p.splits = wd.splits;
    p.qkv = use_u && (E.mode == EPI_QKV_HEADS || (E.mode == EPI_QK_HEADS && E.ln_stats));
    const int cap = cand.grid ? cand.grid : gemm_knobs().force_grid ? gemm_knobs().force_grid : 512;
    p.grid = std::min(wd.n_items, cap);
    p.stats_nb = (E.stats_out && use_u && wd.splits == 1 && A.mode == A_ROWS && E.mode == EPI_ROWMAJOR && !E.out_f32 && E.act != ACT_GEGLU &&
                  E.act != ACT_GELU && E.act != ACT_QUICK_GELU && !(E.res && E.act == ACT_SILU)  &&
                  N % (tn * 16) == 0 && N / (tn * 16) <= E.stats_ld)
                     ? N / (tn * 16) : 0;
    if (E.ln_stats && (!use_u || A.mode != A_ROWS || wd.splits > 1 || (tm == 4 && tn == 5) || (E.mode != EPI_QKV_HEADS && E.mode != EPI_QK_HEADS)))
        return set_error(GL_ERR_UNSUPPORTED, "gemm: the folded-LayerNorm epilogue exists for the head layouts of gemm_u_kernel and the GEGLU form of gemm_wide_kernel");
    if (p.qkv && tm == 4 && tn == 5) return set_error(GL_ERR_UNSUPPORTED, "gemm: no 128x160 tile for EPI_QKV_HEADS");
    const char* red = reduce_suffix(p.splits);
    if (use_u && E.mode == EPI_QKV_HEADS) snprintf(p.name, sizeof p.name, "gemm_u_kernel<2, %d, %d, 0, 2, true>%s", tm, tn, red);
    else if (use_u) snprintf(p.name, sizeof p.name, "gemm_u_kernel<2, %d, %d, %d, 2, false>%s", tm, tn, A.mode, red);
    else snprintf(p.name, sizeof p.name, "gemm_p_kernel<%d, %d, %d>%s", tm, tn, A.mode, red);
    return GL_OK;
}

static std::unordered_map<std::string, GemmCand> g_tuned;
static std::mutex g_tune_mu;

static bool tuned_lookup(const char* key, bool use_u, GemmCand& out) {
    if (g_tuned.empty() && use_u && !gemm_knobs().no_table) {
        static const struct { const char* key; int c, sp, grid; } kTable[] = {
#include "gemm_tuned.inc"
        };
        for (const auto& e : kTable) g_tuned.emplace(e.key, GemmCand{e.c, e.sp, e.grid});
    }
    const auto it = g_tuned.find(key);
    if (it != g_tuned.end()) out = it->second;
    return it != g_tuned.end();
}

int gemm_plan(const AOperand& A, int M, int N, int K, Epilogue& E, bool has_ws, size_t ws_bytes, GemmPlan& p, const GemmTuner& tuner) {
    GL_TRY(gemm_validate(A, M, N, K, E));
    const GemmProblem pb{A, M, N, K, E, has_ws, ws_bytes};
    int Mh = (t_plan_scale > 1 && M <= 0x7fffffff / t_plan_scale) ? M * t_plan_scale : M;
    int family = gemm_route(A, Mh, N, K, E);
    if (Mh != M) {
        const int own = gemm_route(A, M, N, K, E);
        if (family != own && !(family == GEMM_HALO && halo_eligible(A, M, N, K, E)) && !(family == GEMM_WIDE && wide_eligible(A, M, N, K, E))) {
            Mh = M;
            family = own;
        }
    }
    const GemmProblem ph{A, Mh, N, K, E, has_ws, ws_bytes};
    p = GemmPlan{family, 0, 0, A.mode};
    if (p.family == GEMM_GLDS) { plan_glds(pb, ph, p); return GL_OK; }
    if (p.family == GEMM_HALO) { plan_halo(pb, ph, p); return GL_OK; }
    if (p.family == GEMM_WIDE) { plan_wide(pb, ph, p); return GL_OK; }
    const bool use_u = p.family == GEMM_U;
    GemmCand pick;
    if (forced_choice(pb, use_u, pick)) return gemm_plan_tile(pb, use_u, pick, p);
    char key[160];
    tuned_key(ph, use_u, key, sizeof key);
    {
        std::lock_guard<std::mutex> lock(g_tune_mu);
        if (!tuned_lookup(key, use_u, pick)) {
            GemmCand model;
            if (!model_choice(ph, use_u, model)) return set_error(GL_ERR_ARG, "gemm: no tile configuration for M=%d N=%d K=%d", M, N, K);
            pick = model;
            if (tuner && gemm_knobs().autotune && Mh == M) {
                bool cache = false;
                GL_TRY(tuner(pb, use_u, key, model, &pick, &cache));
                if (cache) g_tuned[key] = pick;
            }
        }
    }
    return gemm_plan_tile(pb, use_u, pick, p);
}

}
```

gligen_amd/csrc/kbench.hip:

```cpp
#include <cstdio>
#include <cstdlib>
#include <chrono>
#include <cstring>
#include <functional>
#include <string>
#include <vector>

#include "attention.h"
#include "ffn.h"
#include "gemm.h"
#include "misc.h"
#include "norm.h"

using namespace gl;
#ifdef GL_FFN_ABLATE
namespace gl { void ff_rows_set_ablation(int abl); }
#endif

static hipStream_t cur_s = nullptr;

#define HC(expr)                                                                          \
    do {                                                                                  \
        hipError_t _e = (expr);                                                           \
        if (_e != hipSuccess) {                                                           \
// ... 354 lines not shown
                GC(layernorm_launch(L, cur_s));
                AOperand A;
                aoperand_rows(A, xn, C, C);
                Epilogue E;
                epilogue_defaults(E);
                E.act = ACT_GEGLU; E.geglu16 = gemm_geglu_layout(); E.out = hid; E.ldo = 4 * C; E.bias = bp1;
                GC(gemm_launch(A, wp1, M, 8 * C, C, E, ws, ws_bytes, cur_s));
                AOperand A2;
                aoperand_rows(A2, hid, 4 * C, 4 * C);
                Epilogue E2;
                epilogue_defaults(E2);
                E2.out = post ? t3 : refout; E2.ldo = C; E2.bias = fb2; E2.res = tmid; E2.ldres = C; E2.gate = fgate;
                GC(gemm_launch(A2, w2b, M, C, 4 * C, E2, ws, ws_bytes, cur_s));
                if (post) {
                    AOperand A3;
                    aoperand_rows(A3, t3, C, C);
                    Epilogue E3;
                    epilogue_defaults(E3);
                    E3.out = refout; E3.ldo = C; E3.bias = fbpost; E3.res = xres; E3.ldres = C;
                    GC(gemm_launch(A3, postb, M, C, C, E3, ws, ws_bytes, cur_s));
                }
            };
            const float us_ref = time_us(separate, reps, s);
            us = time_us(relaunch, reps, s);
            {
                float d, m, d2, m2;
                maxdiff(a2, refout, (size_t)M * C, s, &d, &m);
                d2 = m2 = 0.f;
                const bool ok = d <= 0.03f * m + 1e-6f;
                if (!ok) ++n_bad;
                printf("FFNC M%d C%d post%d: one launch %.1f us (%.0f TF/s) vs %d separate launches %.1f us; maxdiff out %g of %g, mid %g of %g %s\n", M, C, post, us,
                       flop / us * 1e-6, 4 + post, us_ref, d, m, d2, m2, ok ? "ok" : "MISMATCH");
            }
        } else if (!strcmp(kind, "conv")) {
            const int B = v[0], H = v[1], W = v[2], C0 = v[3], C1 = v[4], Cout = v[5], stride = v[6], ups = v[7];
            count = v[8]; c = 1;
            const int Hup = H << ups, Wup = W << ups;
            const int Ho = stride == 1 ? Hup : (Hup + 2 - 3) / 2 + 1, Wo = stride == 1 ? Wup : (Wup + 2 - 3) / 2 + 1;
            const int M = B * Ho * Wo, K = 9 * (C0 + C1);
            flop = 2.0 * M * Cout * K;
            gM = M; gN = Cout; gK = K;
            AOperand A{};
            A.p0 = a0; A.C0 = C0; A.ld0 = C0; A.p1 = C1 ? a1 : nullptr; A.C1 = C1; A.ld1 = C1;
            A.mode = A_CONV3; A.Hin = H; A.Win = W; A.Ho = Ho; A.Wo = Wo; A.stride = stride; A.ups = ups; A.pad_lo = 1;
            Epilogue E;
            epilogue_defaults(E);
            E.out = a2; E.ldo = Cout; E.bias = bias; E.bias2 = gam; E.bias2_ld = Cout; E.rows_per_b = Ho * Wo;
            if (Cout == 32) { E.mode = EPI_NCHW_F32; E.n_real = 4; E.bias2 = nullptr; }
            relaunch = [=] { GC(gemm_launch(A, w, M, Cout, K, E, cur_s == s ? ws : ws2, ws_bytes, cur_s)); };
            if (stride == 1 && ups == 1 && !C1 && Cout != 32 && (size_t)C0 * Cout <= (size_t)1280 * 1280) {
                static float* wf = nullptr;
                static bf16 *w9 = nullptr, *w4 = nullptr;
                if (!wf) {
                    wf = dev_f32((size_t)9 * 1280 * 1280, 31, 0.02f);
                    HC(hipMalloc(&w9, (size_t)9 * 1280 * 1280 * 2));
                    HC(hipMalloc(&w4, (size_t)16 * 1280 * 1280 * 2));
                    HC(hipDeviceSynchronize());
                }
                GC(pack_conv_weight_launch(wf, w9, Cout, C0, 3, 3, Cout, s));
                GC(pack_upconv_phases_launch(wf, w4, Cout, C0, Cout, s));
                E.bias2 = nullptr;
                const bf16* w9c = w9;
                relaunch = [=] { GC(gemm_launch(A, w9c, M, Cout, K, E, cur_s == s ? ws : ws2, ws_bytes, cur_s)); };
                AOperand A4 = A;
                A4.mode = A_CONV2UP; A4.ups = 0;
                Epilogue E4 = E;
                E4.out = a1;
                if (gemm_upconv_phases_supported(A4, M, Cout, 4 * C0, E4)) {
                    const bf16* w4c = w4;
                    auto phases = [=] { GC(gemm_launch(A4, w4c, M, Cout, 4 * C0, E4, cur_s == s ? ws : ws2, ws_bytes, cur_s)); };
                    const float us4 = time_us(phases, reps, s);
                    int ptm, ptn, psp;
                    gemm_last_cfg(&ptm, &ptn, &psp);
                    us = time_us(relaunch, reps, s);
                    float d, m;
                    maxdiff(a2, a1, (size_t)M * Cout, s, &d, &m);
                    const bool ok = d <= 0.02f * m + 1e-6f;
                    if (!ok) ++n_bad;
                    printf("UPCONV %-51s %9.1f %9.1f  phase form %dx%d/%d (nine-tap FLOP rate; %.2fx of the nine-tap %.1f us) maxdiff %g of %g %s\n", line, us4,
                           flop / us4 * 1e-6, ptm * 32, ptn * 32, psp, us4 / us, us, d, m, ok ? "ok" : "MISMATCH");
                } else {
                    us = time_us(relaunch, reps, s);
                }
            } else {
                us = time_us(relaunch, reps, s);
            }
        } else if (!strcmp(kind, "gnconv")) {
            const int B = v[0], H = v[1], W = v[2], C0 = v[3], C1 = v[4], Cout = v[5];
            count = v[6]; c = 1;
            const int M = B * H * W, Cin = C0 + C1, K = 9 * Cin;
            flop = 2.0 * M * Cout * K;
            gM = M; gN = Cout; gK = K;
            bf16* y_norm = a2;
            bf16* out1 = a2 + ((size_t)96 << 20);
            bf16* out2 = a2 + ((size_t)160 << 20);
            float* coef = partial + (1 << 17);
            GNParams P{};
            P.x0 = a0; P.C0 = C0; P.x1 = C1 ? a1 : nullptr; P.C1 = C1; P.B = B; P.HW = H * W; P.eps = 1e-5f;
            P.gamma = gam; P.beta = bias; P.y = y_norm; P.silu = 1; P.partial = partial; P.coef = coef;
            AOperand A{};
            A.mode = A_CONV3; A.Hin = H; A.Win = W; A.Ho = H; A.Wo = W; A.stride = 1; A.ups = 0; A.pad_lo = 1;
            Epilogue E;
            epilogue_defaults(E);
            E.ldo = Cout; E.bias = bias; E.bias2 = gam; E.bias2_ld = Cout; E.rows_per_b = H * W;
            AOperand A1 = A, A2 = A;
            A1.p0 = y_norm; A1.C0 = Cin; A1.ld0 = Cin;
            A2.p0 = a0; A2.C0 = C0; A2.ld0 = C0; A2.p1 = C1 ? a1 : nullptr; A2.C1 = C1; A2.ld1 = C1; A2.gn = coef;
            Epilogue E1 = E, E2 = E;
            E1.out = out1; E2.out = out2;
            if (!gemm_gn_prologue_supported(A2, M, Cout, K, E2)) { printf("%-58s no GroupNorm prologue for this shape\n", line); continue; }
            auto two_pass = [=] { GC(groupnorm_launch(P, cur_s)); GC(gemm_launch(A1, w, M, Cout, K, E1, cur_s == s ? ws : ws2, ws_bytes, cur_s)); };
            auto gn_only = [=] { GC(groupnorm_launch(P, cur_s)); };
            auto conv_only = [=] { GC(gemm_launch(A1, w, M, Cout, K, E1, cur_s == s ? ws : ws2, ws_bytes, cur_s)); };
            auto coef_only = [=] { GC(groupnorm_coef_launch(P, cur_s)); };
            auto conv_pro = [=] { GC(gemm_launch(A2, w, M, Cout, K, E2, cur_s == s ? ws : ws2, ws_bytes, cur_s)); };
            relaunch = [=] { GC(groupnorm_coef_launch(P, cur_s)); GC(gemm_launch(A2, w, M, Cout, K, E2, cur_s == s ? ws : ws2, ws_bytes, cur_s)); };
            const float us2 = time_us(two_pass, reps, s);
            us = time_us(relaunch, reps, s);
            const float t_gn = time_us(gn_only, reps, s), t_cv = time_us(conv_only, reps, s), t_cf = time_us(coef_only, reps, s), t_cp = time_us(conv_pro, reps, s);
            float d, m;
            maxdiff(out1, out2, (size_t)M * Cout, s, &d, &m);
            const bool exact = H * W > 256;
            const bool ok = exact ? d == 0.f : d <= 0.01f * m;
            if (!ok) ++n_bad;
            printf("GNCONV %-44s two passes %.1f us (gn %.1f + conv %.1f) | prologue %.1f us (stats %.1f + conv %.1f)  maxdiff %g of %g %s\n", line, us2, t_gn, t_cv,
                   us, t_cf, t_cp, d, m, !ok ? "MISMATCH" : d == 0.f ? "bit-equal" : "within a bf16 step");
        } else if (!strcmp(kind, "attn")) {
            const int B = v[0], H = v[1], d = v[2], Nq = v[3], Nk = v[4];
            count = v[5]; c = 2;
            flop = 4.0 * B * H * d * (double)Nq * Nk;
            int dp, dpv;
            GC(attn_dims(d, &dp, &dpv));
            AttnParams P{};
            P.vt_layout = attn_vt_layout(d, Nk, &dpv);
            P.q = a0; P.k = a1; P.vt = a2;
            bf16* o = a2 + ((size_t)200 << 20);
            P.o = o;
            P.H = H; P.d = d; P.Nq = Nq; P.Nk = Nk; P.Tq_pad = round_up(Nq, 128); P.Tk_pad = round_up(Nk, 64);
            P.ldo = H * d; P.o_rows_per_b = Nq;
            P.scale_log2e = 1.4426950408889634f / sqrtf((float)d);
            GC(attn_vt_ones_launch(a2, B * H, d, P.Tk_pad, s, dpv));
            GC(attn_k_init_launch(a1, B * H, d, P.Tk_pad, s));
            relaunch = [=] { GC(attn_launch(P, B, cur_s)); };
            us = time_us(relaunch, reps, s);
        } else if (!strcmp(kind, "gn")) {
            const int B = v[0], HW = v[1], C0 = v[2], C1 = v[3], silu = v[4];
            count = v[5]; c = 3;
            bytes = 2.0 * B * HW * (double)(C0 + C1) * 2;
            GNParams P{};
            P.x0 = a0; P.C0 = C0; P.x1 = C1 ? a1 : nullptr; P.C1 = C1; P.B = B; P.HW = HW; P.eps = 1e-5f;
            P.gamma = gam; P.beta = bias; P.y = a2; P.silu = silu; P.partial = partial;
            relaunch = [=] { GC(groupnorm_launch(P, cur_s)); };
            us = time_us(relaunch, reps, s);
        } else if (!strcmp(kind, "ln")) {
            const int B = v[0], N1 = v[1], N2 = v[2], Tpad = v[3], C = v[4];
            count = v[5]; c = 4;
            bytes = 2.0 * B * (double)(N1 + N2) * C * 2;
            LNParams P{};
            P.x = a0; P.x2 = N2 ? a1 : nullptr; P.B = B; P.N1 = N1; P.N2 = N2; P.Tpad = Tpad; P.C = C; P.eps = 1e-5f;
            P.gamma = gam; P.beta = bias; P.y = a2;
            relaunch = [=] { GC(layernorm_launch(P, cur_s)); };
            us = time_us(relaunch, reps, s);
        } else {
            continue;
        }
        if (sweep && c <= 1) {
// ... 107 lines not shown
```

gligen_amd/engine.py:

```python
from __future__ import annotations

import ctypes as C
from typing import Dict, Mapping, Optional, Sequence

import numpy as np
import torch

from . import _lib, vae_tiling
from ._lib import Grounding, PlmsArgs, SolverArgs, UNetConfig, VaeConfig, check

GROUNDING_KINDS = {"text": 0, "text_image": 1, "keypoint": 2, "tokens": 3}


def _stream(device=None) -> C.c_void_p:
    return C.c_void_p(torch.cuda.current_stream(device).cuda_stream)


def _ptr(t: Optional[torch.Tensor]) -> C.c_void_p:
    return C.c_void_p(0 if t is None else t.data_ptr())


def _f32(t: torch.Tensor, device) -> torch.Tensor:
    return t.to(device=device, dtype=torch.float32).contiguous()

# ... 691 lines not shown
                raise ValueError(f"op_lora_merge: {name} must be a contiguous fp32 tensor on {self.device} (it is {what})")
            if t.dim() < 2:
                raise ValueError(f"op_lora_merge: {name} has shape {tuple(t.shape)}, need at least two dimensions")
        N, r = int(W.shape[0]), int(down.shape[0])
        K = int(np.prod(W.shape[1:]))
        if int(up.shape[0]) != N or up.numel() != N * r or down.numel() != r * K:
            raise ValueError(f"op_lora_merge: up {tuple(up.shape)} @ down {tuple(down.shape)} does not give W {tuple(W.shape)}")
        check(self.lib.gl_op_lora_merge(self._ctx, _ptr(W), _ptr(up), _ptr(down), N, K, r, float(scale), _stream(self.device)))
        return W

    def sampler_timing(self):
        a, f, n = C.c_float(), C.c_float(), C.c_int()
        check(self.lib.gl_sampler_timing(self._ctx, C.byref(a), C.byref(f), C.byref(n)))
        return float(a.value), float(f.value), int(n.value)

    def to_uint8(self, img: torch.Tensor) -> torch.Tensor:
        img = _f32(img, self.device)
        B, Cc, H, W = img.shape
        out = torch.empty((B, H, W, Cc), device=self.device, dtype=torch.uint8)
        check(self.lib.gl_to_uint8(_ptr(img), _ptr(out), int(B), int(Cc), int(H * W), _stream(self.device)))
        return out

    def arena_high_water(self) -> int:
        v = C.c_size_t()
        check(self.lib.gl_arena_high_water(self._ctx, C.byref(v)))
        return int(v.value)

    def launch_count(self) -> int:
        v = C.c_int64()
        check(self.lib.gl_launch_count(self._ctx, C.byref(v)))
        return int(v.value)

    def box_calibrate(self) -> dict:
        from ._lib import BoxCalibration
        c = BoxCalibration()
        check(self.lib.gl_box_calibrate(self._ctx, C.byref(c), _stream(self.device)))
        return {"hbm_copy_GBps": round(float(c.hbm_copy_gbs), 1), "lds_dma_TBps": round(float(c.lds_dma_tbs), 2),
                "mfma_bf16_TFLOPs": round(float(c.mfma_bf16_tflops), 1)}

    def mfma_calibrate(self, shape: int = 0, waves_per_simd: int = 2, n_acc: int = 4, zero_data: bool = False, target_ms: float = 25.0) -> dict:
        from ._lib import MfmaCalibration
        c = MfmaCalibration()
        check(self.lib.gl_mfma_calibrate(self._ctx, int(shape), int(waves_per_simd), int(n_acc), int(bool(zero_data)), float(target_ms), C.byref(c),
                                         _stream(self.device)))
        return {"shape": "32x32x16" if shape == 0 else "16x16x32", "waves_per_simd": int(waves_per_simd), "accumulators": int(n_acc),
                "data": "zeros" if zero_data else "random", "TFLOPs": round(float(c.tflops), 1), "sclk_MHz": round(float(c.sclk_mhz), 1),
                "ms": round(float(c.ms), 2), "cycles_per_mfma": round(float(c.cycles_per_mfma), 2),
                "frac_of_2.5PF": round(float(c.tflops) / 2500.0, 3)}

    def mfma_calibration_table(self, target_ms: float = 25.0) -> list:
        rows = []
        for shape in (0, 1):
            for wps in (1, 2):
                rows.append(self.mfma_calibrate(shape, wps, 8, False, target_ms))
        rows.append(self.mfma_calibrate(0, 2, 4, False, target_ms))
        rows.append(self.mfma_calibrate(0, 2, 8, True, target_ms))
        return rows

    def set_ff_rows_policy(self, mode: int) -> None:
        check(self.lib.gl_set_ff_rows_policy(int(mode)))

    def set_cfg_shared_prefix(self, on: bool) -> None:
        check(self.lib.gl_set_cfg_shared_prefix(int(bool(on))))

    def gemm_force_plan(self, tm=0, tn=0, splits=0, grid_cap=0) -> None:
        check(self.lib.gl_gemm_force_plan(int(tm), int(tn), int(splits), int(grid_cap)))

    def gemm_force_knobs(self, halo_splits, wide_splits, wide_xcd, xcd_boxes, halo, wide) -> None:
        check(self.lib.gl_gemm_force_knobs(int(halo_splits), int(wide_splits), int(wide_xcd), int(xcd_boxes), int(halo), int(wide)))

    def gemm_force_clear(self) -> None:
        check(self.lib.gl_gemm_force_clear())

    def gemm_plan_log_clear(self) -> None:
        check(self.lib.gl_gemm_plan_log_clear())

    def gemm_plan_log(self):
        from ._lib import GemmPlanRecord
        recs = (GemmPlanRecord * 32)()
        n, total = C.c_int(0), C.c_int(0)
        check(self.lib.gl_gemm_plan_log(recs, 32, C.byref(n), C.byref(total)))
        out = [{f: (getattr(r, f).decode() if f == "kernel" else getattr(r, f)) for f, _ in GemmPlanRecord._fields_} for r in recs[:n.value]]
        return out, total.value

    def ff_rows_policy_report(self) -> str:
        buf = C.create_string_buffer(4096)
        check(self.lib.gl_ff_rows_policy_report(buf, 4096))
        return buf.value.decode()

    def op_linear(self, x, w, bias=None, res=None, act=0, out_f32=False):
        M, K = x.shape
        N = w.shape[0]
        y = torch.empty((M, N), device=x.device, dtype=torch.float32 if out_f32 else torch.bfloat16)
        check(self.lib.gl_op_linear(self._ctx, _ptr(x), _ptr(w), _ptr(bias), _ptr(res), _ptr(y), M, N, K, act, int(out_f32), _stream(self.device)))
        return y

    def op_geglu(self, x, w_f32, b_f32):
        M, K = x.shape
        inner = w_f32.shape[0] // 2
        y = torch.empty((M, inner), device=x.device, dtype=torch.bfloat16)
        check(self.lib.gl_op_geglu(self._ctx, _ptr(x), _ptr(w_f32), _ptr(b_f32), _ptr(y), M, inner, K, _stream(self.device)))
        return y

    def op_ln_linear(self, a, w0, b0, res, gamma, beta, w1, b1, mode, inner_or_heads, T=0):
        M, K0 = a.shape
        Cc = w0.shape[0]
        x = torch.empty((M, Cc), device=a.device, dtype=torch.bfloat16)
        if mode == 0:
            y = torch.empty((M, inner_or_heads), device=a.device, dtype=torch.bfloat16)
        else:
            d = Cc // inner_or_heads
            dp = {40: 48, 80: 80, 160: 160}[d]
            y = torch.zeros((M // T * inner_or_heads, ((T + 127) // 128) * 128, dp), device=a.device, dtype=torch.bfloat16)
        used = C.c_int(-1)
        check(self.lib.gl_op_ln_linear(self._ctx, _ptr(a), M, K0, _ptr(w0), _ptr(b0), _ptr(res), Cc, _ptr(gamma), _ptr(beta), _ptr(w1),
                                       _ptr(b1), int(mode), int(inner_or_heads), int(T), _ptr(x), _ptr(y), C.byref(used), _stream(self.device)))
        return x, y, int(used.value)

    def op_feedforward(self, x, w1, b1, w2, b2, gamma=None, beta=None, res=None, gate=None, want_stats=False):
        M, Cc = x.shape
        y = torch.empty((M, Cc), device=x.device, dtype=torch.bfloat16)
        stats = torch.zeros((M, 2), device=x.device, dtype=torch.float32) if want_stats else None
        used = C.c_int(-1)
        check(self.lib.gl_op_feedforward(self._ctx, _ptr(x), M, Cc, _ptr(gamma), _ptr(beta), _ptr(w1), _ptr(b1), _ptr(w2), _ptr(b2),
                                         _ptr(res), _ptr(gate), _ptr(y), _ptr(stats), C.byref(used), _stream(self.device)))
        return y, stats, int(used.value)

    def op_ff_chain(self, x, pre_w, pre_b, pre_res, gamma, beta, w1, b1, w2, b2, pre_gate=None, gate=None, post_w=None, post_b=None, post_res=None):
        M, Cc = x.shape
        y = torch.empty((M, Cc), device=x.device, dtype=torch.bfloat16)
        check(self.lib.gl_op_ff_chain(self._ctx, _ptr(x), M, Cc, _ptr(pre_w), _ptr(pre_b), _ptr(pre_res), _ptr(pre_gate), _ptr(gamma), _ptr(beta),
                                      _ptr(w1), _ptr(b1), _ptr(w2), _ptr(b2), _ptr(gate), _ptr(post_w), _ptr(post_b), _ptr(post_res), _ptr(y),
                                      _stream(self.device)))
        return y

    def op_adamw_step(self, p, g, m, v, step, lr=5e-5, betas=(0.9, 0.999), eps=1e-8, weight_decay=0.0):
        for t in (p, g, m, v):
            assert t.is_cuda and t.dtype == torch.float32 and t.is_contiguous() and t.numel() == p.numel()
        check(self.lib.gl_op_adamw_step(self._ctx, _ptr(p), _ptr(g), _ptr(m), _ptr(v), p.numel(), float(lr), float(betas[0]), float(betas[1]),
                                        float(eps), float(weight_decay), int(step), _stream(self.device)))

    ADAMW_EMA_GRID = (16384, 256, 4)

    def op_adamw_ema_step(self, p, g, m, v, ema, step, *, ema_rate, lr=5e-5, betas=(0.9, 0.999), eps=1e-8, weight_decay=0.0):
        for t in (p, g, m, v, ema):
            assert t.is_cuda and t.dtype == torch.float32 and t.is_contiguous() and t.numel() == p.numel()
        check(self.lib.gl_op_adamw_ema_step(self._ctx, _ptr(p), _ptr(g), _ptr(m), _ptr(v), _ptr(ema), p.numel(), float(lr), float(betas[0]), float(betas[1]),
                                            float(eps), float(weight_decay), float(ema_rate), int(step), _stream(self.device)))

    GRAD_NORM_GRID = (16384, 64, 6, 4)

    @staticmethod
    def _flat(*ts):
        for t in ts:
            assert t.is_cuda and t.dtype == torch.float32 and t.is_contiguous() and t.numel() == ts[0].numel()

    def op_grad_accumulate(self, acc, g, mode: str, k: int):
        self._flat(acc, g)
        check(self.lib.gl_op_grad_accumulate(self._ctx, _ptr(acc), _ptr(g), g.numel(), _lib.GRAD_ACCUM_MODES[mode], int(k), _stream(self.device)))

    def grad_sqnorm_partials(self, n: int) -> int:
        return int(self.lib.gl_grad_sqnorm_partials(int(n)))

    def op_grad_sqnorm(self, g, partials=None):
        self._flat(g)
        count = self.grad_sqnorm_partials(g.numel())
# ... 631 lines not shown
```

Baseline: 6.838 images/s.

## Add specialized 3x3 conv kernel for 8x8 feature maps with halo tiling

Adds a dedicated conv8_kernel for the 3x3, stride-1, pad-1 convolutions on 8x8 spatial maps in the UNet's lowest-resolution blocks. It stages 256-pixel halo tiles and weight slabs into LDS with buffer-to-LDS DMA and double buffering, then runs MFMA over the three kx taps. A planner picks the column tile (64 or 80) and the split-K count from a small cost model plus measured entries. Engine::gemm now routes eligible A_CONV3 calls to this path automatically. The aim is to cut the im2col overhead and poor occupancy of the generic conv GEMM on these tiny spatial sizes, at the cost of a new hand-scheduled kernel and split-K reduction slabs.

After: 6.916 images/s, median of 6. +1.1%, better.

```diff
diff --git a/gligen_amd/_lib.py b/gligen_amd/_lib.py
--- a/gligen_amd/_lib.py
+++ b/gligen_amd/_lib.py
@@ -292,6 +292,19 @@
 ATTENTION_CORE_SYMBOLS = {
     "gl_op_attention_core": (_I, [_P, _P, _P, _P, C.POINTER(AttnProjLayout), _I, _I, _I, _I, _P, _I, _I, _I, _P]),
 }
+
+
+class Conv8Args(C.Structure):
+    _fields_ = [("struct_size", C.c_uint), ("x0", _P), ("x1", _P)] + [(n, _I) for n in ("C0", "C1", "B", "H", "W", "N", "stride", "ups", "pad_lo")] + \
+               [("w", _P), ("bias", _P), ("bias2", _P), ("bias2_ld", _I), ("rows_per_b", _I), ("res", _P), ("ldres", _I), ("act", _I), ("out_f32", _I),
+                ("out", _P), ("ldo", _I), ("bn", _I), ("splits", _I), ("grid_cap", _I), ("slabs", _P), ("slab_bytes", C.c_size_t)]
+
+
+CONV8_SYMBOLS = {
+    "gl_op_conv8x8": (_I, [_P, C.POINTER(Conv8Args), _P]),
+    "gl_conv8_routed": (_I, [C.POINTER(Conv8Args)]),
+    "gl_conv8_force_knobs": (_I, [_I, _I, _I]),
+}
 ATTN_CORE_KERNELS = {"auto": 0, "attn_kernel": 1, "attn2_kernel_w4": 2, "attn2_kernel_w8": 3, "attn3_kernel": 4}
 GL_ERR_UNSUPPORTED = 5
 
@@ -380,7 +393,7 @@
     import torch
     lib = C.CDLL(str(LIB_PATH))
     for name, (res, args) in {**SYMBOLS, **IMAGE_SYMBOLS, **MAP_SYMBOLS, **TRAIN_MAP_SYMBOLS, **TRAIN_INPUT_SYMBOLS, **TRAIN_FUSER_SYMBOLS, **TRAIN_PRIM_SYMBOLS,
-                              **TRAINER_SYMBOLS, **SAMPLER_SYMBOLS, **SOLVER_SYMBOLS, **GEMM_PLAN_SYMBOLS, **ATTENTION_CORE_SYMBOLS, **FFN_ROWS_SYMBOLS, **NORM_SYMBOLS, **VAE_SYMBOLS, **LATENT_SYMBOLS, **LORA_SYMBOLS, **TILING_SYMBOLS, **TRAIN_LORA_SYMBOLS, **TRAIN_LORA_CONV_SYMBOLS,
+                              **TRAINER_SYMBOLS, **SAMPLER_SYMBOLS, **SOLVER_SYMBOLS, **GEMM_PLAN_SYMBOLS, **ATTENTION_CORE_SYMBOLS, **CONV8_SYMBOLS, **FFN_ROWS_SYMBOLS, **NORM_SYMBOLS, **VAE_SYMBOLS, **LATENT_SYMBOLS, **LORA_SYMBOLS, **TILING_SYMBOLS, **TRAIN_LORA_SYMBOLS, **TRAIN_LORA_CONV_SYMBOLS,
                               **TRAIN_RUN_SYMBOLS}.items():
         fn = getattr(lib, name)
         fn.restype = res
diff --git a/gligen_amd/build.py b/gligen_amd/build.py
--- a/gligen_amd/build.py
+++ b/gligen_amd/build.py
@@ -11,7 +11,7 @@
 CSRC = HERE / "csrc"
 INCLUDE = HERE.parent / "include"
 LIB = HERE / "libgligen_amd.so"
-GEMM_UNITS = ["gemm_u.hip", "gemm_halo.hip", "gemm_wide.hip", "gemm_basic.hip", "gemm.hip"]
+GEMM_UNITS = ["gemm_u.hip", "gemm_halo.hip", "gemm_wide.hip", "gemm_conv8.hip", "gemm_basic.hip", "gemm.hip"]
 SOURCES = [*GEMM_UNITS, "gemm_plan.hip", "ffn.hip", "attention.hip", "vae_attention.hip", "clip.hip", "norm.hip", "misc.hip", "image.hip", "latent.hip", "tile.hip", "lora.hip", "classmap.hip", "convnext.hip",
            "train_ops.hip", "train_attention.hip", "train_layers.hip", "train_spatial.hip", "train_unet.hip", "train_inputs.hip", "train_fusers.hip", "train_optim.hip", "train_lora.hip", "train_lora_conv.hip", "train_run.hip",
            "engine.hip", "engine_unet.hip", "engine_policy.hip", "engine_vae.hip", "engine_clip.hip", "engine_spatial.hip", "engine_sampler.hip", "capi.hip"]
diff --git a/gligen_amd/csrc/capi.hip b/gligen_amd/csrc/capi.hip
--- a/gligen_amd/csrc/capi.hip
+++ b/gligen_amd/csrc/capi.hip
@@ -18,6 +18,7 @@
 #include "../../include/gligen_amd_sampler.h"
 #include "../../include/gligen_amd_gemm_plans.h"
 #include "../../include/gligen_amd_attention_core.h"
+#include "../../include/gligen_amd_conv8.h"
 #include "../../include/gligen_amd_ffn_rows.h"
 #include "../../include/gligen_amd_norm.h"
 #include "../../include/gligen_amd_vae.h"
@@ -563,6 +564,7 @@
         r.family = p.family; r.M = e[i].M; r.N = e[i].N; r.K = e[i].K;
         r.tm = p.tm; r.tn = p.tn; r.splits = p.splits; r.grid = p.grid;
         if (p.family == GEMM_HALO) { r.n_items = p.halo.n_items; r.units_per_split = p.halo.chunks_per_split; }
+        else if (p.family == GEMM_CONV8) { r.n_items = p.conv8.n_items; r.units_per_split = p.conv8.chunks_per_split; }
         else if (p.family == GEMM_WIDE) { r.n_items = p.wide.n_items; r.units_per_split = p.wide.kt_per_split; r.xcd = p.wide.xcd; }
         else {
             r.n_items = p.work.n_items; r.units_per_split = p.work.kt_per_split;
@@ -1641,6 +1643,60 @@
     GL_API_END
 }
 
+static bool conv8_describe(const gl_conv8_args* a, AOperand& A, Epilogue& E, int& M, int& K) {
+    if (a->C0 < 1 || a->C1 < 0 || a->B < 1 || a->H < 1 || a->W < 1 || a->N < 1 || a->ups < 0 || a->ups > 1 || (a->stride != 1 && a->stride != 2) ||
+        a->rows_per_b < 1)
+        return false;
+    const int Cin = a->C0 + a->C1;
+    const int Hup = a->H << a->ups, Wup = a->W << a->ups;
+    const int Ho = a->stride == 1 ? Hup : (a->pad_lo ? (Hup + 2 - 3) / 2 + 1 : (Hup + 1 - 3) / 2 + 1);
+    const int Wo = a->stride == 1 ? Wup : (a->pad_lo ? (Wup + 2 - 3) / 2 + 1 : (Wup + 1 - 3) / 2 + 1);
+    A = AOperand{};
+    A.p0 = (const bf16*)a->x0; A.C0 = a->C0; A.ld0 = a->C0; A.p1 = (const bf16*)a->x1; A.C1 = a->C1; A.ld1 = a->C1;
+    A.mode = A_CONV3; A.Hin = a->H; A.Win = a->W; A.Ho = Ho; A.Wo = Wo; A.stride = a->stride; A.ups = a->ups; A.pad_lo = a->pad_lo;
+    M = a->B * Ho * Wo; K = 9 * Cin;
+    epilogue_defaults(E);
+    E.act = a->act; E.out = a->out; E.ldo = a->ldo; E.out_f32 = a->out_f32;
+    E.bias = a->bias; E.bias2 = a->bias2; E.bias2_ld = a->bias2_ld; E.rows_per_b = a->rows_per_b;
+    E.res = (const bf16*)a->res; E.ldres = a->ldres;
+    return true;
+}
+int gl_conv8_routed(const gl_conv8_args* a) {
+    if (!a || a->struct_size != sizeof(gl_conv8_args)) { gl::set_error(GL_ERR_ARG, "gl_conv8_routed: null args or a struct_size that is not this library's"); return -1; }
+    AOperand A;
+    Epilogue E;
+    int M, K;
+    if (!conv8_describe(a, A, E, M, K)) { gl::set_error(GL_ERR_ARG, "gl_conv8_routed: conv geometry"); return -1; }
+    return gemm_conv8_supported(A, M, a->N, K, E) ? 1 : 0;
+}
+int gl_conv8_force_knobs(int on, int bn, int splits) {
+    if (on < 0 || on > 1 || (bn != 0 && bn != 64 && bn != 80) || splits < 0 || splits > 32)
+        return gl::set_error(GL_ERR_ARG, "gl_conv8_force_knobs: on %d, bn %d, splits %d (0 | 1, 0 | 64 | 80, 0..32)", on, bn, splits);
+    gemm_conv8_force_knobs(on, bn, splits);
+    return GL_OK;
+}
+int gl_op_conv8x8(gl_ctx* ctx, const gl_conv8_args* a, gl_stream s) {
+    NEED(ctx);
+    if (!a) return gl::set_error(GL_ERR_ARG, "gl_op_conv8x8: null args");
+    if (a->struct_size != sizeof(gl_conv8_args))
+        return gl::set_error(GL_ERR_ARG, "gl_op_conv8x8: args->struct_size is %u, this library's gl_conv8_args has %zu bytes", a->struct_size, sizeof(gl_conv8_args));
+    if (!a->x0 || !a->w || !a->out || (a->C1 && !a->x1) || (a->splits > 1 && !a->slabs))
+        return gl::set_error(GL_ERR_ARG, "gl_op_conv8x8: null pointer (x0, w, out; x1 when C1 > 0; slabs when splits > 1)");
+    GL_API_BEGIN
+    AOperand A;
+    Epilogue E;
+    int M, K;
+    if (!conv8_describe(a, A, E, M, K)) throw GlError(GL_ERR_ARG, "gl_op_conv8x8: conv geometry");
+    Arena& ar = ctx->eng->arena();
+    ar.reset();
+    bf16* wp = ar.get<bf16>((size_t)a->N * K);
+    int r = pack_conv_weight_launch((const float*)a->w, wp, a->N, a->C0 + a->C1, 3, 3, a->N, S(s));
+    if (r != GL_OK) throw GlError(r, gl::last_error());
+    r = gemm_conv8_launch(A, wp, M, a->N, K, E, a->splits > 1 ? a->slabs : nullptr, a->splits > 1 ? a->slab_bytes : 0, a->bn, a->splits, a->grid_cap, S(s));
+    if (r != GL_OK) throw GlError(r, gl::last_error());
+    GL_API_END
+}
+
 int gl_op_attention_core(gl_ctx* ctx, const void* q, const void* k, const void* vt, const gl_attn_proj_layout* layout, int B, int H, int Nq,
                          int Nk, void* o, int ldo, int o_rows_per_b, int kernel, gl_stream s) {
     NEED(ctx);
diff --git a/gligen_amd/csrc/engine.hip b/gligen_amd/csrc/engine.hip
--- a/gligen_amd/csrc/engine.hip
+++ b/gligen_amd/csrc/engine.hip
@@ -488,8 +488,10 @@
     ++n_launches;
 }
 
-void Engine::gemm(const AOperand& A, const bf16* W, int M, int N, int K, const Epilogue& E, hipStream_t s) {
+void Engine::gemm(const AOperand& A_in, const bf16* W, int M, int N, int K, const Epilogue& E, hipStream_t s) {
     ProfScope ps(this, s, "gemm", 2.0 * M * N * K, 0.0);
+    AOperand A = A_in;
+    if (A.mode == A_CONV3 && gemm_conv8_supported(A, M, N, K, E)) A.mode = A_CONV8;
     CK(gemm_launch(A, W, M, N, K, E, ws_, ws_bytes_, s));
     if (profiling_) {
         static const bool by_shape = dev_env("GL_PROF_SHAPES") != nullptr;
diff --git a/gligen_amd/csrc/gemm.h b/gligen_amd/csrc/gemm.h
--- a/gligen_amd/csrc/gemm.h
+++ b/gligen_amd/csrc/gemm.h
@@ -3,7 +3,7 @@
 
 namespace gl {
 
-enum { A_ROWS = 0, A_CONV3 = 1, A_CONV2UP = 2 };
+enum { A_ROWS = 0, A_CONV3 = 1, A_CONV2UP = 2, A_CONV8 = 3 };
 
 struct AOperand {
     const bf16* p0;
@@ -79,6 +79,9 @@
 bool gemm_gn_prologue_supported(const AOperand& A, int M, int N, int K, const Epilogue& E);
 bool gemm_upconv_phases_supported(const AOperand& A, int M, int N, int K, const Epilogue& E);
 bool gemm_ln_fold_supported(const AOperand& A, int M, int N, int K, const Epilogue& E);
+bool gemm_conv8_supported(const AOperand& A, int M, int N, int K, const Epilogue& E);
+int gemm_conv8_launch(const AOperand& A, const bf16* W, int M, int N, int K, const Epilogue& E, float* ws, size_t ws_bytes, int bn, int splits,
+                      int grid_cap, hipStream_t stream);
 int gemm_last_stats_nb();
 void aoperand_rows(AOperand& A, const bf16* p, int K, int ld);
 
diff --git a/gligen_amd/csrc/gemm.hip b/gligen_amd/csrc/gemm.hip
--- a/gligen_amd/csrc/gemm.hip
+++ b/gligen_amd/csrc/gemm.hip
@@ -133,6 +133,7 @@
         case GEMM_U: GL_TRY(gemm_exec_u(l, p)); break;
         case GEMM_HALO: GL_TRY(gemm_exec_halo(l, p)); break;
         case GEMM_WIDE: GL_TRY(gemm_exec_wide(l, p)); break;
+        case GEMM_CONV8: GL_TRY(gemm_exec_conv8(l, p)); break;
         default: return gemm_unknown_tile();
     }
     if (p.splits > 1) {
@@ -210,6 +211,18 @@
     return execute(plan, A, W, M, N, K, E, ws, stream);
 }
 
+int gemm_conv8_launch(const AOperand& A_in, const bf16* W, int M, int N, int K, const Epilogue& E_in, float* ws, size_t ws_bytes, int bn, int splits,
+                      int grid_cap, hipStream_t stream) {
+    t_last.stats_nb = 0;
+    AOperand A = A_in;
+    A.mode = A_CONV8;
+    Epilogue E = E_in;
+    GemmPlan plan;
+    GL_TRY(gemm_conv8_plan(A, M, N, K, E, ws != nullptr, ws_bytes, bn, splits, grid_cap, plan));
+    t_last = plan;
+    return execute(plan, A, W, M, N, K, E, ws, stream);
+}
+
 int gemm_launch_t(const bf16* Wrows, int Mw, const bf16* X, int Nx, int K, const Epilogue& E, hipStream_t stream) {
     AOperand A;
     aoperand_rows(A, Wrows, K, K);
diff --git a/gligen_amd/csrc/gemm_conv8.hip b/gligen_amd/csrc/gemm_conv8.hip
--- /dev/null
+++ b/gligen_amd/csrc/gemm_conv8.hip
@@ -0,0 +1,196 @@
+#include "gemm_impl.h"
+
+namespace gl {
+
+template <int TNF>
+__global__ void __launch_bounds__(512, 1)
+conv8_kernel(AOperand A, const bf16* __restrict__ W, int M, int N, int K, Epilogue E, float* __restrict__ ws, Conv8Desc cd) {
+    constexpr int BN = TNF * 16;
+    constexpr int HSTR = 90;
+    constexpr int HROWS = 4 * HSTR + 10;
+    constexpr int HBUF = HROWS * 128;
+    constexpr int WROWS = 3 * BN;
+    constexpr int WSLOT = WROWS * 128;
+    constexpr int WP = (WROWS + 63) / 64;
+    constexpr unsigned SENT = 0x80000000u;
+    static_assert(WROWS % 8 == 0 && BN % 8 == 0, "a wave's eight DMA rows share one kx");
+
+    extern __shared__ __attribute__((aligned(16))) unsigned char smem[];
+
+    const int t = threadIdx.x;
+    const int lane = t & 63;
+    const int wave = __builtin_amdgcn_readfirstlane(t >> 6);
+    const int l15 = lane & 15;
+    const int q = lane >> 4;
+    const int Cin = A.C0 + A.C1;
+    const int nchunks = Cin >> 6;
+    const unsigned lds0 = (unsigned)(uintptr_t)(__attribute__((address_space(3))) unsigned char*)smem;
+
+    const __amdgpu_buffer_rsrc_t ra0 = __builtin_amdgcn_make_buffer_rsrc((void*)A.p0, 0, 0x80000000u, 0x00020000);
+    const __amdgpu_buffer_rsrc_t ra1 = __builtin_amdgcn_make_buffer_rsrc((void*)(A.p1 ? A.p1 : A.p0), 0, 0x80000000u, 0x00020000);
+    const __amdgpu_buffer_rsrc_t rw = __builtin_amdgcn_make_buffer_rsrc((void*)W, 0, 0x80000000u, 0x00020000);
+
+    for (int o = t * 16; o < 2 * HBUF; o += 512 * 16) *reinterpret_cast<uint4*>(smem + o) = make_uint4(0u, 0u, 0u, 0u);
+    __syncthreads();
+
+    const int px = lane >> 3;
+    const unsigned chb_h = (unsigned)(((lane & 7) ^ ((((px + 1) >> 1) & 3) << 1)) * 16);
+    int w_kx[WP], w_n[WP];
+#pragma unroll
+    for (int i = 0; i < WP; ++i) {
+        const int R = i * 64 + (t >> 3);
+        w_kx[i] = R / BN;
+        w_n[i] = R - w_kx[i] * BN;
+    }
+
+    const int sm = wave >> 1, half = wave & 1;
+    unsigned afrag[3];
+#pragma unroll
+    for (int kx = 0; kx < 3; ++kx) {
+        const int X = (l15 & 7) + kx;
+        const int hr = sm * HSTR + (half * 4 + (l15 >> 3)) * 10 + X;
+        afrag[kx] = lds0 + (unsigned)(hr * 128 + ((q ^ (((X >> 1) & 3) << 1)) << 4));
+    }
+    const unsigned wfrag = lds0 + 2 * HBUF + (unsigned)(l15 * 128 + ((q ^ (l15 >> 1)) << 4));
+
+    f32x4 acc[2][TNF];
+
+    for (int item = blockIdx.x; item < cd.n_items; item += gridDim.x) {
+        const int n_u = cd.tiles_n * cd.splits;
+        const int G = 8 * cd.tiles_m;
+        const int g = item / G, rem = item - g * G;
+        const int width = min(8, n_u - g * 8);
+        const int tm = rem / width;
+        const int u = g * 8 + (rem - tm * width);
+        const int c_tn = u / cd.splits;
+        const int c_z = u - c_tn * cd.splits;
+        const int m0 = tm * 256;
+        const int ch0 = c_z * cd.chunks_per_split;
+        const int ch1 = min(nchunks, ch0 + cd.chunks_per_split);
+        const int nstages = (ch1 - ch0) * 3;
+
+        unsigned vw[WP];
+#pragma unroll
+        for (int i = 0; i < WP; ++i)
+            vw[i] = ((unsigned)(c_tn * BN + w_n[i]) * (unsigned)K + (unsigned)(w_kx[i] * Cin)) * 2u + (unsigned)(((t & 7) ^ ((w_n[i] >> 1) & 7)) * 16);
+
+        auto issue_pixels = [&](int ch_, int hb_) {
+            const int ch = __builtin_amdgcn_readfirstlane(ch_);
+            const int hb = __builtin_amdgcn_readfirstlane(hb_);
+            const int cc = ch * 64;
+            const bool first = cc < A.C0;
+            const unsigned ld2 = (unsigned)(first ? A.ld0 : A.ld1) * 2u;
+            const int soff = (first ? cc : cc - A.C0) * 2;
+#pragma unroll
+            for (int p = 0; p < 4; ++p) {
+                const int m = m0 + p * 64 + (t >> 3);
+                const unsigned va = m < M ? (unsigned)m * ld2 + chb_h : SENT;
+                unsigned char* dst = smem + hb * HBUF + (p * HSTR + (wave + 1) * 10 + 1) * 128;
+                if (first) GL_BLDS16(ra0, dst, va, soff);
+                else GL_BLDS16(ra1, dst, va, soff);
+            }
+        };
+        auto issue_w = [&](int st_, int wsl_) {
+            const int st = __builtin_amdgcn_readfirstlane(st_);
+            const int wsl = __builtin_amdgcn_readfirstlane(wsl_);
+            const int dch = st / 3, ky = st - dch * 3;
+            const int soff = (ky * 3 * Cin + (ch0 + dch) * 64) * 2;
+            unsigned char* dst = smem + 2 * HBUF + wsl * WSLOT + wave * 1024;
+#pragma unroll
+            for (int i = 0; i < WP; ++i) {
+                if (i * 64 + wave * 8 >= WROWS) continue;
+                GL_BLDS16(rw, dst + i * 64 * 128, vw[i], soff);
+            }
+        };
+
+        auto tap = [&](auto KX, unsigned aoff, unsigned woff) {
+            constexpr int kx = decltype(KX)::value;
+            const unsigned ax0 = afrag[kx] + aoff, ax1 = ax0 ^ 64u;
+            const unsigned aw0 = wfrag + woff + kx * BN * 128, aw1 = aw0 ^ 64u;
+            bf16x8 xa[2], wa[TNF], xb[2], wb[TNF];
+            lds_rd16<0>(xa[0], ax0);
+            lds_rd16<2560>(xa[1], ax0);
+            lds_rd16_n<TNF, 2048>(wa, aw0);
+            lds_rd16<0>(xb[0], ax1);
+            lds_rd16<2560>(xb[1], ax1);
+            lds_rd16_n<TNF, 2048>(wb, aw1);
+            asm volatile("s_waitcnt lgkmcnt(%0)" ::"n"(2 + TNF));
+            pin_regs(xa);
+            pin_regs(wa);
+            __builtin_amdgcn_sched_barrier(0);
+#pragma unroll
+            for (int i = 0; i < 2; ++i)
+#pragma unroll
+                for (int j = 0; j < TNF; ++j) acc[i][j] = __builtin_amdgcn_mfma_f32_16x16x32_bf16(wa[j], xa[i], acc[i][j], 0, 0, 0);
+            asm volatile("s_waitcnt lgkmcnt(0)");
+            pin_regs(xb);
+            pin_regs(wb);
+            __builtin_amdgcn_sched_barrier(0);
+#pragma unroll
+            for (int i = 0; i < 2; ++i)
+#pragma unroll
+                for (int j = 0; j < TNF; ++j) acc[i][j] = __builtin_amdgcn_mfma_f32_16x16x32_bf16(wb[j], xb[i], acc[i][j], 0, 0, 0);
+        };
+
+#pragma unroll
+        for (int i = 0; i < 2; ++i)
+#pragma unroll
+            for (int j = 0; j < TNF; ++j) acc[i][j] = f32x4{0.f, 0.f, 0.f, 0.f};
+
+        __builtin_amdgcn_s_barrier();
+        asm volatile("" ::: "memory");
+        issue_pixels(ch0, 0);
+        issue_w(0, 0);
+        int st = 0;
+#pragma unroll 1
+        for (int dch = 0; dch < ch1 - ch0; ++dch) {
+            const int hb = dch & 1;
+#pragma unroll 1
+            for (int ky = 0; ky < 3; ++ky, ++st) {
+                const int wsl = st & 1;
+                __builtin_amdgcn_s_waitcnt(0x0F70);
+                __builtin_amdgcn_s_barrier();
+                asm volatile("" ::: "memory");
+                if (st + 1 < nstages) issue_w(st + 1, wsl ^ 1);
+                if (ky == 0 && ch0 + dch + 1 < ch1) issue_pixels(ch0 + dch + 1, hb ^ 1);
+                const unsigned aoff = (unsigned)(hb * HBUF + ky * 1280), woff = (unsigned)(wsl * WSLOT);
+                tap(std::integral_constant<int, 0>{}, aoff, woff);
+                tap(std::integral_constant<int, 1>{}, aoff, woff);
+                tap(std::integral_constant<int, 2>{}, aoff, woff);
+            }
+        }
+
+        const int mrow = m0 + sm * 64 + half * 32 + l15;
+        const int ncol = c_tn * BN + q * 4;
+        if (m0 + sm * 64 < M) {
+#pragma unroll
+            for (int i = 0; i < 2; ++i) {
+                const int m = mrow + i * 16;
+#pragma unroll
+                for (int j = 0; j < TNF; ++j) {
+                    const int n0 = ncol + j * 16;
+                    if (cd.splits > 1) {
+                        *reinterpret_cast<float4*>(ws + ((size_t)c_z * M + m) * N + n0) = make_float4(acc[i][j][0], acc[i][j][1], acc[i][j][2], acc[i][j][3]);
+                    } else {
+                        float v[4] = {acc[i][j][0], acc[i][j][1], acc[i][j][2], acc[i][j][3]};
+                        epi_finish4(E, m, n0, v);
+                    }
+                }
+            }
+        }
+    }
+}
+
+namespace {
+constexpr size_t conv8_lds(int tnf) { return 2 * 370 * 128 + 2 * 3 * tnf * 16 * 128; }
+}
+
+int gemm_exec_conv8(const Launch& l, const GemmPlan& p) {
+    switch (p.tn) {
+        case 4: return l.run<conv8_kernel<4>>(p.grid, 512, conv8_lds(4), p.conv8);
+        case 5: return l.run<conv8_kernel<5>>(p.grid, 512, conv8_lds(5), p.conv8);
+    }
+    return gemm_unknown_tile();
+}
+
+}
diff --git a/gligen_amd/csrc/gemm_impl.h b/gligen_amd/csrc/gemm_impl.h
--- a/gligen_amd/csrc/gemm_impl.h
+++ b/gligen_amd/csrc/gemm_impl.h
@@ -285,6 +285,7 @@
 int gemm_exec_u(const Launch& l, const GemmPlan& p);
 int gemm_exec_halo(const Launch& l, const GemmPlan& p);
 int gemm_exec_wide(const Launch& l, const GemmPlan& p);
+int gemm_exec_conv8(const Launch& l, const GemmPlan& p);
 inline int gemm_unknown_tile() { return set_error(GL_ERR_UNSUPPORTED, "gemm: unknown tile candidate"); }
 
 }
diff --git a/gligen_amd/csrc/gemm_plan.h b/gligen_amd/csrc/gemm_plan.h
--- a/gligen_amd/csrc/gemm_plan.h
+++ b/gligen_amd/csrc/gemm_plan.h
@@ -21,6 +21,10 @@
     int tiles_n, splits, kt_per_split, n_items;
     int xcd;
 };
+struct Conv8Desc {
+    int tiles_n, splits, chunks_per_split, n_items;
+    int tiles_m;
+};
 
 struct GemmKnobs {
     int variant = 4;
@@ -30,10 +34,12 @@
     int autotune = 1, tune_reps = 3, corun = 0;
     bool no_table = false, tune_log = false;
     int force_tm = 0, force_tn = 0, force_splits = 0, force_grid = 0;
+    int conv8 = 1, conv8_bn = 0, conv8_splits = 0;
 };
 GemmKnobs& gemm_knobs();
 void gemm_force_knobs(int halo_splits, int wide_splits, int wide_xcd, int xcd_boxes, int halo, int wide);
 void gemm_force_clear();
+void gemm_conv8_force_knobs(int on, int bn, int splits);
 
 struct GemmProblem {
     const AOperand& A;
@@ -42,7 +48,7 @@
     bool has_ws; size_t ws_bytes;
 };
 
-enum GemmFamily { GEMM_GLDS, GEMM_P, GEMM_U, GEMM_HALO, GEMM_WIDE };
+enum GemmFamily { GEMM_GLDS, GEMM_P, GEMM_U, GEMM_HALO, GEMM_WIDE, GEMM_CONV8 };
 
 struct GemmCand { int c, sp, grid; };
 constexpr int kGemmTiles = 5;
@@ -54,7 +60,7 @@
     bool qkv, gn;
     int splits;
     int grid;
-    union { WorkDesc work; HaloDesc halo; WideDesc wide; };
+    union { WorkDesc work; HaloDesc halo; WideDesc wide; Conv8Desc conv8; };
     int stats_nb;
     char name[96];
 };
@@ -71,4 +77,6 @@
 
 int gemm_plan(const AOperand& A, int M, int N, int K, Epilogue& E, bool has_ws, size_t ws_bytes, GemmPlan& plan, const GemmTuner& tuner = nullptr);
 
+int gemm_conv8_plan(const AOperand& A, int M, int N, int K, Epilogue& E, bool has_ws, size_t ws_bytes, int bn, int splits, int grid_cap, GemmPlan& plan);
+
 }
diff --git a/gligen_amd/csrc/gemm_plan.hip b/gligen_amd/csrc/gemm_plan.hip
--- a/gligen_amd/csrc/gemm_plan.hip
+++ b/gligen_amd/csrc/gemm_plan.hip
@@ -14,7 +14,8 @@
         {"GL_GEMM_VARIANT", &GemmKnobs::variant}, {"GL_GEMM_WIDE", &GemmKnobs::wide}, {"GL_GEMM_WIDE_SPLITS", &GemmKnobs::wide_splits},
         {"GL_CONV_HALO", &GemmKnobs::halo}, {"GL_CONV_HALO_SPLITS", &GemmKnobs::halo_splits}, {"GL_GEMM_XCD_BOXES", &GemmKnobs::xcd_boxes},
         {"GL_WIDE_XCD", &GemmKnobs::wide_xcd}, {"GL_GEMM_AUTOTUNE", &GemmKnobs::autotune}, {"GL_GEMM_TUNE_REPS", &GemmKnobs::tune_reps},
-        {"GL_GEMM_TUNE_CORUN", &GemmKnobs::corun}};
+        {"GL_GEMM_TUNE_CORUN", &GemmKnobs::corun}, {"GL_CONV8", &GemmKnobs::conv8}, {"GL_CONV8_BN", &GemmKnobs::conv8_bn},
+        {"GL_CONV8_SPLITS", &GemmKnobs::conv8_splits}};
     GemmKnobs k;
     for (const auto& e : kInt)
         if (const char* v = dev_env(e.env)) k.*e.knob = atoi(v);
@@ -35,11 +36,16 @@
     GemmKnobs& k = gemm_knobs();
     k.halo_splits = halo_splits; k.wide_splits = wide_splits; k.wide_xcd = wide_xcd; k.xcd_boxes = xcd_boxes; k.halo = halo; k.wide = wide;
 }
+void gemm_conv8_force_knobs(int on, int bn, int splits) {
+    GemmKnobs& k = gemm_knobs();
+    k.conv8 = on; k.conv8_bn = bn; k.conv8_splits = splits;
+}
 void gemm_force_clear() {
     const GemmKnobs d = read_knobs();
     gemm_force_cfg(0, 0, 0);
     gemm_force_grid(0);
     gemm_force_knobs(d.halo_splits, d.wide_splits, d.wide_xcd, d.xcd_boxes, d.halo, d.wide);
+    gemm_conv8_force_knobs(d.conv8, d.conv8_bn, d.conv8_splits);
 }
 static thread_local int t_no_split = 0;
 void gemm_set_no_split(int on) { t_no_split = on; }
@@ -73,6 +79,21 @@
     if (E.bias2 && (E.rows_per_b != A.Hin * A.Win)) return false;
     return fits_buffer_offsets(A, M, N, K);
 }
+static bool conv8_kernel_eligible(const AOperand& A, int M, int N, int K, const Epilogue& E) {
+    if ((A.mode != A_CONV3 && A.mode != A_CONV8) || A.stride != 1 || A.ups || A.pad_lo != 1 || A.gn) return false;
+    if (A.Hin != 8 || A.Win != 8 || A.Ho != 8 || A.Wo != 8 || M <= 0 || M % 64) return false;
+    if (A.C0 <= 0 || A.C0 % 64 || A.C1 % 64 || K != 9 * (A.C0 + A.C1) || (N % 64 && N % 80)) return false;
+    if (E.mode != EPI_ROWMAJOR || E.remap_in || E.gate || (E.act != ACT_NONE && E.act != ACT_SILU) || E.ln_stats) return false;
+    return fits_buffer_offsets(A, M, N, K);
+}
+bool gemm_conv8_supported(const AOperand& A, int M, int N, int K, const Epilogue& E) {
+    const GemmKnobs& kn = gemm_knobs();
+    if (!kn.conv8 || kn.variant != 4 || kn.force_tm || A.C0 + A.C1 < 640 || N < 128 || (E.bias2 && E.res)) return false;
+    if (kn.conv8_bn && (kn.conv8_bn != 64 && kn.conv8_bn != 80)) return false;
+    if (kn.conv8_bn && N % kn.conv8_bn) return false;
+    return conv8_kernel_eligible(A, M, N, K, E);
+}
+
 static bool wide_eligible(const AOperand& A, int M, int N, int K, const Epilogue& E) {
     if (A.mode != A_ROWS || M % 256 || (N % 160 && N % 128)) return false;
     if (A.C1 && A.C0 % 64) return false;
@@ -84,6 +105,7 @@
 
 static int gemm_route(const AOperand& A, int M, int N, int K, const Epilogue& E, bool honour_force = true) {
     const GemmKnobs& kn = gemm_knobs();
+    if (A.mode == A_CONV8) return GEMM_CONV8;
     if (A.mode == A_CONV2UP) return kn.variant == 4 && fits_buffer_offsets(A, M, N, K) ? GEMM_U : GEMM_P;
     if (kn.variant < 2 || (N < 128 && E.act != ACT_GEGLU)) return GEMM_GLDS;
     const bool use_u = kn.variant == 4 && fits_buffer_offsets(A, M, N, K) && !(E.bias2 && (E.res || A.mode == A_ROWS));
@@ -134,6 +156,9 @@
     if (A.mode == A_CONV2UP) {
         if (!gemm_upconv_phases_supported(A, M, N, K, E))
             return set_error(GL_ERR_UNSUPPORTED, "conv3x3: no phase form of the upsample conv for this launch (gemm_u_kernel, bias-only bf16 epilogue, K = 4 Cin, N %% 8 == 0)");
+    } else if (A.mode == A_CONV8) {
+        if (!conv8_kernel_eligible(A, M, N, K, E))
+            return set_error(GL_ERR_UNSUPPORTED, "conv3x3: A_CONV8 is the 3x3 / stride 1 / pad 1 conv of 8 x 8 images (channels %% 64, N %% 64 or 80, plain row-major epilogue)");
     } else if (A.mode == A_CONV3) {
         if ((A.C0 + A.C1) % 64 != 0 || A.C0 % 64 != 0 || K != 9 * (A.C0 + A.C1))
             return set_error(GL_ERR_ARG, "conv3x3: channels (%d,%d) must be multiples of 64 and K=9*Cin (K=%d)", A.C0, A.C1, K);
@@ -233,6 +258,46 @@
     p.tm = 8; p.tn = tn; p.splits = wd.splits;
     p.grid = std::min(wd.n_items, 256);
     snprintf(p.name, sizeof p.name, "gemm_wide_kernel<%d>%s", tn, reduce_suffix(p.splits));
+}
+
+void plan_conv8_choice(const GemmProblem& ph, int& bn, int& splits) {
+    const int N = ph.N, chunks = (ph.A.C0 + ph.A.C1) / 64, groups = cdiv(ph.M, 256);
+    const GemmKnobs& kn = gemm_knobs();
+    static const struct { int M, N, chunks, bn, sp; } kMeasured[] = {{512, 1280, 20, 64, 5}, {512, 1280, 40, 80, 8}};
+    int want_bn = kn.conv8_bn, want_sp = kn.conv8_splits;
+    if (!kn.no_table)
+        for (const auto& e : kMeasured)
+            if (e.M == ph.M && e.N == N && e.chunks == chunks) {
+                if (!want_bn && !want_sp) { want_bn = e.bn; want_sp = e.sp; }
+            }
+    double best = 1e300;
+    bn = 0; splits = 1;
+    for (int b = 64; b <= 80; b += 16) {
+        if (N % b || (want_bn && want_bn != b)) continue;
+        const int tiles = groups * (N / b);
+        for (int sp = 1; sp <= std::min(chunks, 32); ++sp) {
+            const int per = cdiv(chunks, sp);
+            if (cdiv(chunks, per) != sp) continue;
+            if (want_sp && sp != cdiv(chunks, cdiv(chunks, std::min(want_sp, chunks)))) continue;
+            if (sp > 1 && (!ph.has_ws || (size_t)sp * ph.M * N * sizeof(float) > ph.ws_bytes)) continue;
+            const double t = cdiv(tiles * sp, 256) * (per * b / 64.0 + 1.0) + (sp > 1 ? 0.5 + 0.25 * sp : 0.0);
+            if (t < best) { best = t; bn = b; splits = sp; }
+        }
+    }
+    if (!bn) { bn = N % 64 == 0 ? 64 : 80; splits = 1; }
+}
+void plan_conv8_fill(const GemmProblem& pb, int bn, int splits, int grid_cap, GemmPlan& p) {
+    const int chunks = (pb.A.C0 + pb.A.C1) / 64;
+    Conv8Desc& cd = p.conv8;
+    cd.tiles_m = cdiv(pb.M, 256);
+    cd.tiles_n = pb.N / bn;
+    cd.chunks_per_split = cdiv(chunks, splits);
+    cd.splits = cdiv(chunks, cd.chunks_per_split);
+    cd.n_items = cd.tiles_m * cd.tiles_n * cd.splits;
+    p.family = GEMM_CONV8;
+    p.tm = 8; p.tn = bn / 16; p.amode = A_CONV8; p.splits = cd.splits;
+    p.grid = std::min(cd.n_items, grid_cap > 0 ? grid_cap : 256);
+    snprintf(p.name, sizeof p.name, "conv8_kernel<%d>%s", bn, reduce_suffix(p.splits));
 }
 
 }
@@ -400,6 +465,13 @@
     if (p.family == GEMM_GLDS) { plan_glds(pb, ph, p); return GL_OK; }
     if (p.family == GEMM_HALO) { plan_halo(pb, ph, p); return GL_OK; }
     if (p.family == GEMM_WIDE) { plan_wide(pb, ph, p); return GL_OK; }
+    if (p.family == GEMM_CONV8) {
+        if (!gemm_conv8_supported(A, M, N, K, E)) return set_error(GL_ERR_UNSUPPORTED, "conv3x3: A_CONV8 without gemm_conv8_supported()");
+        int bn, splits;
+        plan_conv8_choice(ph, bn, splits);
+        plan_conv8_fill(pb, bn, splits, gemm_knobs().force_grid, p);
+        return GL_OK;
+    }
     const bool use_u = p.family == GEMM_U;
     GemmCand pick;
     if (forced_choice(pb, use_u, pick)) return gemm_plan_tile(pb, use_u, pick, p);
@@ -421,4 +493,18 @@
     return gemm_plan_tile(pb, use_u, pick, p);
 }
 
-}
+int gemm_conv8_plan(const AOperand& A, int M, int N, int K, Epilogue& E, bool has_ws, size_t ws_bytes, int bn, int splits, int grid_cap, GemmPlan& p) {
+    if (A.mode != A_CONV8) return set_error(GL_ERR_ARG, "gemm_conv8_plan: the operand is not A_CONV8");
+    GL_TRY(gemm_validate(A, M, N, K, E));
+    const int chunks = (A.C0 + A.C1) / 64;
+    if ((bn != 64 && bn != 80) || N % bn || splits < 1 || splits > chunks || cdiv(chunks, cdiv(chunks, splits)) != splits || grid_cap < 0)
+        return set_error(GL_ERR_ARG, "conv8: column tile %d / %d splits of %d chunks / cap %d (tile 64 | 80 dividing N, every part with a chunk, cap >= 0)", bn, splits, chunks, grid_cap);
+    if (splits > 1 && (!has_ws || (size_t)splits * M * N * sizeof(float) > ws_bytes))
+        return set_error(GL_ERR_ARG, "conv8: %d slabs of %d x %d do not fit the workspace", splits, M, N);
+    const GemmProblem pb{A, M, N, K, E, has_ws, ws_bytes};
+    p = GemmPlan{GEMM_CONV8, 0, 0, A.mode};
+    plan_conv8_fill(pb, bn, splits, grid_cap, p);
+    return GL_OK;
+}
+
+}
diff --git a/gligen_amd/csrc/kbench.hip b/gligen_amd/csrc/kbench.hip
--- a/gligen_amd/csrc/kbench.hip
+++ b/gligen_amd/csrc/kbench.hip
@@ -460,6 +460,22 @@
                 } else {
                     us = time_us(relaunch, reps, s);
                 }
+            } else if (gemm_conv8_supported(A, M, Cout, K, E)) {
+                AOperand A8 = A;
+                A8.mode = A_CONV8;
+                Epilogue E8 = E;
+                if (!C1) E8.out = a1;
+                auto conv8 = [=] { GC(gemm_launch(A8, w, M, Cout, K, E8, cur_s == s ? ws : ws2, ws_bytes, cur_s)); };
+                const float us8 = time_us(conv8, reps, s);
+                int ptm, ptn, psp;
+                gemm_last_cfg(&ptm, &ptn, &psp);
+                us = time_us(relaunch, reps, s);
+                float d = 0.f, m = 0.f;
+                if (!C1) maxdiff(a2, a1, (size_t)M * Cout, s, &d, &m);
+                const bool ok = d <= 0.02f * m + 1e-6f;
+                if (!ok) ++n_bad;
+                printf("CONV8  %-51s %9.1f %9.1f  conv8_kernel<%d>/%d (%.2fx of gemm_u_kernel's %.1f us) maxdiff %g of %g %s\n", line, us8, flop / us8 * 1e-6,
+                       ptn * 16, psp, us8 / us, us, d, m, ok ? "ok" : "MISMATCH");
             } else {
                 us = time_us(relaunch, reps, s);
             }
diff --git a/gligen_amd/engine.py b/gligen_amd/engine.py
--- a/gligen_amd/engine.py
+++ b/gligen_amd/engine.py
@@ -797,6 +797,25 @@
         check(self.lib.gl_gemm_plan_log(recs, 32, C.byref(n), C.byref(total)))
         out = [{f: (getattr(r, f).decode() if f == "kernel" else getattr(r, f)) for f, _ in GemmPlanRecord._fields_} for r in recs[:n.value]]
         return out, total.value
+
+    def conv8_force_knobs(self, on=1, bn=0, splits=0) -> None:
+        check(self.lib.gl_conv8_force_knobs(int(on), int(bn), int(splits)))
+
+    def op_conv8x8(self, x0, w, out, bn, splits, *, x1=None, bias=None, bias2=None, rows_per_b=64, res=None, act=0, slabs=None, grid_cap=0,
+                   B=None, ldo=None):
+        from ._lib import Conv8Args
+        a = Conv8Args()
+        a.struct_size = C.sizeof(Conv8Args)
+        a.x0 = _ptr(x0); a.x1 = _ptr(x1)
+        a.C0 = x0.shape[-1]; a.C1 = 0 if x1 is None else x1.shape[-1]
+        a.B = x0.shape[0] if B is None else B
+        a.H = a.W = 8; a.N = w.shape[0]; a.stride = 1; a.ups = 0; a.pad_lo = 1
+        a.w = _ptr(w); a.bias = _ptr(bias); a.bias2 = _ptr(bias2); a.bias2_ld = a.N; a.rows_per_b = rows_per_b
+        a.res = _ptr(res); a.ldres = a.N; a.act = act; a.out_f32 = int(out.dtype == torch.float32)
+        a.out = _ptr(out); a.ldo = a.N if ldo is None else ldo
+        a.bn = bn; a.splits = splits; a.grid_cap = grid_cap
+        a.slabs = _ptr(slabs); a.slab_bytes = 0 if slabs is None else slabs.numel() * 4
+        check(self.lib.gl_op_conv8x8(self._ctx, C.byref(a), _stream(self.device)))
 
     def ff_rows_policy_report(self) -> str:
         buf = C.create_string_buffer(4096)
diff --git a/include/gligen_amd_conv8.h b/include/gligen_amd_conv8.h
--- /dev/null
+++ b/include/gligen_amd_conv8.h
@@ -0,0 +1,39 @@
+#ifndef GLIGEN_AMD_CONV8_H
+#define GLIGEN_AMD_CONV8_H
+#include <stddef.h>
+
+#include "gligen_amd.h"
+
+#ifdef __cplusplus
+extern "C" {
+#endif
+
+typedef struct gl_conv8_args {
+    unsigned struct_size;
+    const void* x0;
+    const void* x1;
+    int C0, C1, B, H, W, N, stride, ups, pad_lo;
+    const void* w;
+    const float* bias;
+    const float* bias2;
+    int bias2_ld, rows_per_b;
+    const void* res;
+    int ldres;
+    int act, out_f32;
+    void* out;
+    int ldo;
+    int bn, splits, grid_cap;
+    float* slabs;
+    size_t slab_bytes;
+} gl_conv8_args;
+
+int gl_conv8_routed(const gl_conv8_args* args);
+
+int gl_op_conv8x8(gl_ctx* ctx, const gl_conv8_args* args, gl_stream s);
+
+int gl_conv8_force_knobs(int on, int bn, int splits);
+
+#ifdef __cplusplus
+}
+#endif
+#endif
```
